# mkeeter/fidget

Measured on AMD Instinct MI355X. Metric: Mvoxel/s (interval+point eval) on prospero.vm 1024^3, higher is better.
Workload: dtype f32; 1 GPU; prospero.vm 3D heightmap+normals 1024^3, HipShape render hints (the library's tiles: 128/32/8, or 32/8 when the root level has few tiles), world_to_model=I

## Files before the change

fidget_amd/__init__.py:

```python
import ctypes as C
import math
import os
import re
import subprocess
import sys

import numpy as np

_HERE = os.path.dirname(os.path.abspath(__file__))
_CSRC = os.path.join(_HERE, "csrc")
LIB_PATH = os.environ.get("FHIP_LIB") or os.path.join(_CSRC, "libfidget_hip.so")
_SOURCES = ["capi.hip", "capi_core.hpp", "capi_context.hpp", "capi_tapes.hpp", "capi_eval.hpp", "capi_render.hpp", "frame_plan.hpp", "frame_schedule.hpp", "capi_effects.hpp", "capi_mesh.hpp", "capi_debug.hpp", "capi_solve.hpp", "solve.hip", "solve_lm.hpp", "kernels.hip", "prune2.hip", "effects.hip", "mesh.hip", "mesh_qef.hpp", "mesh_collapse.hpp", "mesh_edges.hpp", "mesh_walk.hpp", "mesh_split.hpp", "mesh_vox.hpp", "mesh_cc.hpp", "mesh_edt.hpp", "edt.hip", "capi_edt.hpp", "mesh_vmesh.hpp", "vmesh.hip", "capi_vmesh.hpp", "contour/contour.hpp", "host_mesh.hpp", "dev_ops.hpp", "host_graph.hpp", "host_regtape.hpp", "render_state.h", "tape_format.h",
            "gen_interp.py", "gen_tiles.py", "gen_tilesv.py", "gen_normals.py", "gen_prune.py", "gen_ubench.py", "gen_trans.py", "trans_funcs.hip", "trans_libm.hpp", "offsets.cpp", "../../include/fidget_hip.h",
            "../../include/fidget_hip_debug.h"]

UNARY = ["neg", "abs", "recip", "sqrt", "square", "floor", "ceil", "round", "sin", "cos", "tan",
         "asin", "acos", "atan", "exp", "ln", "not", "rand"]
BINARY = ["add", "sub", "mul", "div", "atan2", "min", "max", "compare", "mod", "and", "or", "mix"]

FH_OPS = (["Output", "Input", "CopyReg", "CopyImm"] + [u.capitalize() for u in UNARY]
          + [b.capitalize() + "RR" for b in ["add", "sub", "mul", "div", "atan2", "compare", "mix", "mod", "min", "max", "and", "or"]]
          + [b.capitalize() + "RI" for b in ["add", "sub", "mul", "div", "atan2", "compare", "mix", "mod", "min", "max", "and", "or"]]
          + [b.capitalize() + "IR" for b in ["sub", "div", "atan2", "compare", "mix", "mod"]])

STATUS = {1: "BadVarSlice", 2: "MismatchedSlices", 3: "BadChoiceSlice", 4: "MissingVar", 5: "BadTape",
          6: "Unsupported", 7: "HipError", 8: "Cancelled", 9: "ParseError", 10: "Overflow"}

VM_TILES_3D = [128, 64, 32, 16, 8]
VM_TILES_2D = [128, 32, 8]
GEOMETRY_PIXEL = np.dtype([("normal", np.float32, 3), ("depth", np.uint32)])
HIP_TILES_2D, HIP_TILES_3D = [128, 16], [128, 32, 8]
VM_TILES_2D, VM_TILES_3D = [128, 32, 8], [128, 64, 32, 16, 8]

EXPORTS = [
    "fhip_ctx_create", "fhip_ctx_destroy", "fhip_ctx_trim", "fhip_ctx_reserve_arena", "fhip_libm_probe", "fhip_last_error", "fhip_ctx_sync", "fhip_cancel", "fhip_cancel_reset", "fhip_cancel_watch", "fhip_ctx_set_option", "fhip_ctx_get_option",
    "fhip_tape_from_bytecode", "fhip_tape_free", "fhip_tape_len", "fhip_tape_reg_tape", "fhip_tape_choice_count", "fhip_tape_reg_count",
    "fhip_tape_var_count", "fhip_tape_output_count", "fhip_tape_ops", "fhip_simplify", "fhip_interval_eval",
    "fhip_point_eval", "fhip_float_eval", "fhip_grad_eval", "fhip_solve", "fhip_render2d", "fhip_render3d", "fhip_render3d_shard", "fhip_render3d_block", "fhip_merge_depth", "fhip_denoise_normals", "fhip_compute_ssao", "fhip_blur_ssao", "fhip_apply_shading", "fhip_to_rgba", "fhip_mesh_sample", "fhip_mesh_build", "fhip_mesh_vertices", "fhip_mesh_triangles", "fhip_mesh_vertices_ptr", "fhip_mesh_triangles_ptr", "fhip_mesh_free", "fhip_mesh_counts", "fhip_mesh_leaves", "fhip_mesh_sample_part", "fhip_mesh_part_bytes", "fhip_mesh_part_export", "fhip_mesh_merge", "fhip_mesh_vertices_dev", "fhip_mesh_triangles_dev", "fhip_mesh_stl_bytes", "fhip_mesh_stl", "fhip_mesh_vertex_grads", "fhip_shape_occupancy", "fhip_voxels_words", "fhip_shape_voxels", "fhip_voxels_slices", "fhip_voxels_layer_counts",
    "fhip_contour2d", "fhip_contours_counts", "fhip_contours_vertices", "fhip_contours_segments", "fhip_contours_next", "fhip_contours_vertices_dev", "fhip_contours_segments_dev", "fhip_contours_free", "fhip_contour_loops",
    "fhip_voxels_components", "fhip_components_counts", "fhip_components_table", "fhip_components_label_slices", "fhip_components_extract", "fhip_components_free",
    "fhip_voxels_distance", "fhip_distance_info", "fhip_distance_slices", "fhip_distance_dev", "fhip_distance_threshold", "fhip_distance_free",
    "fhip_voxels_surface", "fhip_voxels_mesh",
    "fhip_profile_enable", "fhip_profile_read", "fhip_profile_read_kernels", "fhip_render_counters", "fhip_graph_new", "fhip_graph_free",
    "fhip_graph_len", "fhip_graph_var", "fhip_graph_constant", "fhip_graph_unary", "fhip_graph_binary",
    "fhip_graph_from_text", "fhip_tape_from_graph", "fhip_tape_axis_slot", "fhip_tape_var_slot",
    "fhip_screen_to_world", "fhip_debug_groups", "fhip_debug_ubench", "fhip_debug_math_sweep", "fhip_debug_stats", "fhip_debug_leaf_stats", "fhip_debug_tape_links", "fhip_debug_tape_chain", "fhip_debug_bench", "fhip_debug_leaves", "fhip_debug_arena", "fhip_debug_probe", "fhip_debug_trans_probe", "fhip_debug_bound_tape", "fhip_debug_lane_frames", "fhip_debug_rare_frames", "fhip_debug_lane_tune", "fhip_debug_walk_dual", "fhip_debug_stl_pack", "fhip_tape_group_count", "fhip_tape_group_op",
    "fhip_tape_group", "fhip_tape_term_plan", "fhip_tape_term_group", "fhip_tape_term_tree", "fhip_tape_term_choice_src",
]


class FidgetHipError(RuntimeError):
    def __init__(self, status, msg=""):
        self.status = status
        super().__init__(f"{STATUS.get(status, status)}: {msg}")


def build(force=False, verbose=False):
    srcs = [os.path.join(_CSRC, s) for s in _SOURCES]
    if os.environ.get("FHIP_LIB"):
        return LIB_PATH
    if not force and os.path.exists(LIB_PATH) and all(os.path.getmtime(s) <= os.path.getmtime(LIB_PATH) for s in srcs):
        return LIB_PATH
    gen = os.path.join(_CSRC, "_gen")
    os.makedirs(gen, exist_ok=True)
    llvm = os.path.join(os.environ.get("ROCM_PATH", "/opt/rocm"), "lib", "llvm", "bin")
    co = os.path.join(gen, "interp_gfx950.co")

    def run(cmd, **kw):
        if verbose:
            print(" ".join(cmd))
        subprocess.check_call(cmd, **kw)

    run(["g++", "-std=c++17", "-I", _CSRC, os.path.join(_CSRC, "offsets.cpp"), "-o", os.path.join(gen, "offsets")])
    with open(os.path.join(gen, "offsets.json"), "w") as f:
        subprocess.check_call([os.path.join(gen, "offsets")], stdout=f)
    ll = os.path.join(gen, "trans_funcs.ll")
    run(["hipcc", "--offload-arch=gfx950", "-O3", "-std=c++17", "-ffp-contract=off", "-S", "-emit-llvm", "--cuda-device-only", "-I", _CSRC,
         "-o", ll, os.path.join(_CSRC, "trans_funcs.hip")])
    ir = open(ll).read()
    groups = set()
    for fn in ("fh_t_sin", "fh_t_atan2", "fh_t_mod", "fh_t_sin4", "fh_t_ln4"):
        m = re.search(rf"^define [^\n]*@{fn}\([^\n]*\) (#\d+)", ir, re.M)
        assert m, f"trans_funcs.ll: {fn} not found"
        groups.add(m.group(1))
    for g in groups:
        ir, n = re.subn(rf"^attributes {g} = {{ ", f'attributes {g} = {{ "amdgpu-num-sgpr"="18" ', ir, flags=re.M)
        assert n == 1
    with open(ll, "w") as f:
        f.write(ir)
    run([os.path.join(llvm, "llc"), "-mtriple=amdgcn-amd-amdhsa", "-mcpu=gfx950", "-O3", "-o", os.path.join(gen, "trans_funcs.s"), ll])
    run([sys.executable, os.path.join(_CSRC, "gen_interp.py"), os.path.join(gen, "offsets.json"),
         os.path.join(gen, "interp_gfx950.s"), os.path.join(gen, "trans_funcs.s")])
    run([os.path.join(llvm, "clang"), "-x", "assembler", "-target", "amdgcn-amd-amdhsa", "-mcpu=gfx950", "-c",
         os.path.join(gen, "interp_gfx950.s"), "-o", os.path.join(gen, "interp_gfx950.o")])
    run([os.path.join(llvm, "ld.lld"), "-shared", os.path.join(gen, "interp_gfx950.o"), "-o", co])
    run(["hipcc", "--offload-arch=gfx950", "-O3", "-std=c++17", "-ffp-contract=off", "-fPIC", "-shared",
         f'-DFH_INTERP_CO="{co}"', "-o", LIB_PATH, os.path.join(_CSRC, "capi.hip")])
    return LIB_PATH


class _Cfg2D(C.Structure):
    _fields_ = [("width", C.c_uint32), ("height", C.c_uint32), ("world_to_model", C.c_void_p), ("z", C.c_float),
                ("pixel_perfect", C.c_int), ("tile_sizes", C.c_void_p), ("n_tile_sizes", C.c_uint32),
                ("var_keys", C.c_void_p), ("var_values", C.c_void_p), ("n_vars", C.c_uint32),
                ("axis_slots", C.c_void_p)]


class _Cfg3D(C.Structure):
    _fields_ = [("width", C.c_uint32), ("height", C.c_uint32), ("depth", C.c_uint32), ("world_to_model", C.c_void_p),
                ("tile_sizes", C.c_void_p), ("n_tile_sizes", C.c_uint32), ("var_keys", C.c_void_p),
                ("var_values", C.c_void_p), ("n_vars", C.c_uint32), ("axis_slots", C.c_void_p)]


_lib = None


def lib():
    global _lib
    if _lib is None:
        if not os.path.exists(LIB_PATH):
            raise ImportError(f"{LIB_PATH} is missing: run `python -c 'import __graft_entry__ as g; g.build()'`")
        L = C.CDLL(LIB_PATH)
        vp, u32, i32, f32, u64 = C.c_void_p, C.c_uint32, C.c_int, C.c_float, C.c_uint64
        sig = {
            "fhip_ctx_create": (i32, [i32, vp, C.POINTER(vp)]), "fhip_ctx_destroy": (None, [vp]),
            "fhip_libm_probe": (i32, [C.c_char_p, C.c_size_t]), "fhip_ctx_trim": (i32, [vp]), "fhip_ctx_reserve_arena": (i32, [vp, C.c_size_t]),
            "fhip_last_error": (C.c_char_p, [vp]), "fhip_ctx_sync": (i32, [vp]),
            "fhip_cancel": (None, [vp]), "fhip_cancel_reset": (None, [vp]), "fhip_cancel_watch": (None, [vp, vp]),
            "fhip_ctx_set_option": (i32, [vp, C.c_char_p, i32]), "fhip_ctx_get_option": (i32, [vp, C.c_char_p, C.POINTER(i32)]),
            "fhip_tape_from_bytecode": (i32, [vp, vp, C.c_size_t, C.POINTER(vp)]), "fhip_tape_free": (None, [vp]),
            "fhip_tape_len": (u32, [vp]), "fhip_tape_reg_tape": (i32, [vp, u32, vp, u32, vp, u32, vp]), "fhip_tape_choice_count": (u32, [vp]), "fhip_tape_reg_count": (u32, [vp]),
            "fhip_tape_var_count": (u32, [vp]), "fhip_tape_output_count": (u32, [vp]),
            "fhip_tape_ops": (u32, [vp, vp, u32]),
            "fhip_simplify": (i32, [vp, vp, vp, u32, C.POINTER(vp)]),
            "fhip_interval_eval": (i32, [vp, vp, vp, u32, u32, vp, vp, vp]),
            "fhip_point_eval": (i32, [vp, vp, vp, u32, u32, vp, vp, vp]),
            "fhip_float_eval": (i32, [vp, vp, vp, vp, u32, vp]),
            "fhip_grad_eval": (i32, [vp, vp, vp, vp, u32, vp]),
            "fhip_solve": (i32, [vp, vp, u32, vp, vp, vp, u32, vp, u32, u32, vp, vp, vp, vp]),
            "fhip_render2d": (i32, [vp, vp, C.POINTER(_Cfg2D), vp, i32]),
            "fhip_render3d": (i32, [vp, vp, C.POINTER(_Cfg3D), vp, i32]),
            "fhip_render3d_shard": (i32, [vp, vp, C.POINTER(_Cfg3D), vp, i32, u32, u32]),
            "fhip_render3d_block": (i32, [vp, vp, C.POINTER(_Cfg3D), vp, i32, u32, vp]),
            "fhip_merge_depth": (i32, [vp, vp, vp, u64, u32]),
            "fhip_denoise_normals": (i32, [vp, vp, u32, u32, vp, i32]),
            "fhip_compute_ssao": (i32, [vp, vp, u32, u32, u32, vp, u32, vp, u32, vp, i32]),
            "fhip_blur_ssao": (i32, [vp, vp, u32, u32, vp, i32]),
            "fhip_apply_shading": (i32, [vp, vp, u32, u32, u32, vp, vp, i32]),
            "fhip_to_rgba": (i32, [vp, vp, u32, u32, i32, vp, i32]),
            "fhip_mesh_sample": (i32, [vp, vp, u32, vp, vp, vp, vp, u32, C.POINTER(vp)]), "fhip_mesh_free": (None, [vp]),
            "fhip_mesh_counts": (None, [vp, vp]), "fhip_mesh_leaves": (None, [vp, vp]),
            "fhip_mesh_build": (i32, [vp, vp, u32, vp, vp, vp, vp, u32, C.POINTER(vp)]),
            "fhip_mesh_vertices": (None, [vp, vp]), "fhip_mesh_triangles": (None, [vp, vp]),
            "fhip_mesh_vertices_ptr": (vp, [vp]), "fhip_mesh_triangles_ptr": (vp, [vp]),
            "fhip_mesh_sample_part": (i32, [vp, vp, u32, vp, vp, vp, vp, u32, u32, u32, C.POINTER(vp)]),
            "fhip_mesh_part_bytes": (C.c_uint64, [vp]), "fhip_mesh_part_export": (None, [vp, vp]),
            "fhip_mesh_merge": (i32, [vp, vp, vp, u32, vp, C.POINTER(vp)]),
            "fhip_mesh_vertices_dev": (vp, [vp]), "fhip_mesh_triangles_dev": (vp, [vp]),
            "fhip_mesh_stl_bytes": (u64, [vp]), "fhip_mesh_stl": (i32, [vp, vp, vp, i32]),
            "fhip_mesh_vertex_grads": (i32, [vp, vp, vp, vp, vp, vp, u32, vp, i32]),
            "fhip_shape_occupancy": (i32, [vp, vp, u32, vp, vp, vp, vp, u32, vp]),
            "fhip_voxels_words": (u64, [u32]), "fhip_shape_voxels": (i32, [vp, vp, u32, vp, vp, vp, vp, u32, vp, i32, vp]),
            "fhip_voxels_slices": (i32, [vp, vp, u32, u32, u32, vp, i32]), "fhip_voxels_layer_counts": (i32, [vp, vp, u32, vp, i32]),
            "fhip_contour2d": (i32, [vp, vp, vp, vp]), "fhip_contours_counts": (None, [vp, vp]), "fhip_contours_vertices": (i32, [vp, vp]),
            "fhip_contours_segments": (i32, [vp, vp]), "fhip_contours_next": (i32, [vp, vp]), "fhip_contours_vertices_dev": (vp, [vp]),
            "fhip_contours_segments_dev": (vp, [vp]), "fhip_contours_free": (None, [vp]), "fhip_contour_loops": (i32, [vp, u64, vp, vp, vp, vp]),
            "fhip_voxels_components": (i32, [vp, vp, u32, i32, u32, i32, vp]), "fhip_components_counts": (None, [vp, vp]),
            "fhip_components_table": (i32, [vp, vp, vp, vp, vp, vp]), "fhip_components_label_slices": (i32, [vp, vp, vp, i32, u32, u32, vp, i32]),
            "fhip_components_extract": (i32, [vp, vp, vp, i32, vp, u64, vp, i32]), "fhip_components_free": (None, [vp]),
            "fhip_voxels_distance": (i32, [vp, vp, u32, i32, i32, vp]), "fhip_distance_info": (None, [vp, vp]), "fhip_distance_slices": (i32, [vp, vp, u32, u32, vp, i32]),
            "fhip_distance_dev": (vp, [vp]), "fhip_distance_threshold": (i32, [vp, vp, u32, i32, vp, i32]), "fhip_distance_free": (None, [vp]),
            "fhip_voxels_surface": (i32, [vp, vp, u32, i32, vp]), "fhip_voxels_mesh": (i32, [vp, vp, u32, i32, vp]),
            "fhip_debug_stl_pack": (i32, [vp, vp, u64, vp, u64, vp]),
            "fhip_profile_enable": (None, [vp, i32]), "fhip_profile_read": (i32, [vp, vp, vp]), "fhip_profile_read_kernels": (i32, [vp, vp, vp]),
            "fhip_render_counters": (i32, [vp, vp]),
            "fhip_debug_stats": (i32, [vp, vp]), "fhip_debug_leaf_stats": (i32, [vp, vp]), "fhip_debug_tape_links": (u32, [vp, vp, u32]), "fhip_debug_tape_chain": (u32, [vp, vp, u32]),
            "fhip_tape_group_count": (u32, [vp]), "fhip_tape_group_op": (i32, [vp]),
            "fhip_tape_group": (i32, [vp, vp, u32, vp]), "fhip_tape_term_plan": (u32, [vp, vp]), "fhip_tape_term_group": (i32, [vp, vp, u32, vp]),
            "fhip_tape_term_tree": (u32, [vp, vp, u32]), "fhip_tape_term_choice_src": (u32, [vp, vp, u32]),
            "fhip_debug_leaves": (u32, [vp, vp, u32]), "fhip_debug_arena": (u32, [vp, u32, u32, vp]), "fhip_debug_probe": (i32, [vp, vp]),
            "fhip_debug_bench": (i32, [vp, vp, u32, u32, i32, vp]),
            "fhip_debug_walk_dual": (None, [vp, u64, vp, vp, u64, i32, vp, vp, vp]),
            "fhip_debug_groups": (u32, [vp, i32, u32, vp, u32, vp]),
            "fhip_debug_ubench": (i32, [vp, u32, u32, u32, vp]),
            "fhip_debug_math_sweep": (i32, [vp, i32, u32, u32, u64, vp, vp]),
            "fhip_debug_trans_probe": (i32, [vp, u32, u32, u32, u64, vp]),
            "fhip_debug_lane_frames": (u64, [vp]),
            "fhip_debug_rare_frames": (u64, [vp]),
            "fhip_debug_lane_tune": (i32, [vp, vp, vp]),
            "fhip_debug_bound_tape": (i32, [vp, vp, vp, vp, vp, u32, C.POINTER(vp)]),
            "fhip_graph_new": (vp, []), "fhip_graph_free": (None, [vp]), "fhip_graph_len": (u32, [vp]),
            "fhip_graph_var": (u32, [vp, i32, u64]), "fhip_graph_constant": (u32, [vp, f32]),
            "fhip_graph_unary": (u32, [vp, i32, u32]), "fhip_graph_binary": (u32, [vp, i32, u32, u32]),
            "fhip_graph_from_text": (u32, [vp, C.c_char_p]),
            "fhip_tape_from_graph": (i32, [vp, vp, vp, u32, C.POINTER(vp)]),
            "fhip_tape_axis_slot": (i32, [vp, i32]), "fhip_tape_var_slot": (i32, [vp, u64]),
            "fhip_screen_to_world": (None, [vp, i32, vp]),
        }
        for name, (res, args) in sig.items():
            fn = getattr(L, name)
            fn.restype = res
            fn.argtypes = args
        _lib = L
    return _lib


def _p(a):
    return a.ctypes.data_as(C.c_void_p) if a is not None else None


class HipContext:

    def __init__(self, device=0, stream=None):
        h = C.c_void_p()
        st = lib().fhip_ctx_create(device, C.c_void_p(stream or 0), C.byref(h))
        if st != 0:
            raise FidgetHipError(st, "no usable HIP device: fidget_amd has no CPU fallback")
        self._h = h

    def __del__(self):
        try:
            lib().fhip_ctx_destroy(self._h)
        except Exception:
            pass

    def check(self, st):
        if st != 0:
            raise FidgetHipError(st, (lib().fhip_last_error(self._h) or b"").decode())

    def sync(self):
        self.check(lib().fhip_ctx_sync(self._h))

    def trim(self):
        self.check(lib().fhip_ctx_trim(self._h))

    def reserve_arena(self, megabytes):
        self.check(lib().fhip_ctx_reserve_arena(self._h, int(megabytes)))

    def cancel(self):
        lib().fhip_cancel(self._h)

    def cancel_watch(self, flag):
        self._watched = flag
        lib().fhip_cancel_watch(self._h, None if flag is None else flag.ctypes.data_as(C.c_void_p))

    def cancel_reset(self):
        lib().fhip_cancel_reset(self._h)

    def lane_tune(self):
        ms, ln = (C.c_float * 3)(), C.c_int(0)
        ph = lib().fhip_debug_lane_tune(self._h, ms, C.byref(ln))
        return {"phase": int(ph), "stage_pipeline_ms": [float(ms[0]), float(ms[2])], "frame_lanes_ms": float(ms[1]), "kept": "frame lanes" if ln.value else "stage pipeline"}

    def lane_frames(self):
        return int(lib().fhip_debug_lane_frames(self._h))

    def rare_frames(self):
        return int(lib().fhip_debug_rare_frames(self._h))

    def set_option(self, name, value=1):
        self.check(lib().fhip_ctx_set_option(self._h, name.encode(), int(value)))

    def option(self, name):
        v = C.c_int(0)
        self.check(lib().fhip_ctx_get_option(self._h, name.encode(), C.byref(v)))
        return v.value

    def options(self, **kw):
        import contextlib

        @contextlib.contextmanager
        def scope():
            old = {k: self.option(k) for k in kw}
            try:
                for k, v in kw.items():
                    self.set_option(k, v)
                yield self
            finally:
                for k, v in old.items():
                    self.set_option(k, v)
        return scope()

    def profile(self, on):
        lib().fhip_profile_enable(self._h, int(on))

    def profile_read(self):
        ms = np.zeros(4, np.float64)
        n = np.zeros(4, np.uint32)
        self.check(lib().fhip_profile_read(self._h, _p(ms), _p(n)))
        names = ["tiles", "points", "normals", "other"]
        return {k: (float(ms[i]), int(n[i])) for i, k in enumerate(names)}

    def profile_read_kernels(self):
        ms = np.zeros(8, np.float64)
        n = np.zeros(8, np.uint32)
        self.check(lib().fhip_profile_read_kernels(self._h, _p(ms), _p(n)))
        names = ["fh_columns", "fh_float_eval_16x4", "fh_float_eval_32x2", "fh_tiles", "fh_prune1", "fh_tiles_v32", "fh_tiles_v64", "unused"]
        return {k: (float(ms[i]), int(n[i])) for i, k in enumerate(names)}

    def counters(self):
        c = np.zeros(8, np.uint64)
        self.check(lib().fhip_render_counters(self._h, _p(c)))
        return {"arena_ops": int(c[0]), "arena_overflow": int(c[1]), "leaves_last_slab": int(c[2]),
                "queue_overflow": int(c[3]), "groups_last_slab": [int(v) for v in c[4:6]], "hip_tile_stage_frames": int(c[6]), "substituted_tile_lists": int(c[7])}

    def last_leaves(self, cap=1 << 20):
        dt = np.dtype([("off", np.uint32), ("len", np.uint32), ("regs", np.uint16), ("choices", np.uint16),
                       ("x", np.uint32), ("y", np.uint32), ("z", np.uint32)])
        buf = np.zeros(cap, dt)
        n = lib().fhip_debug_leaves(self._h, _p(buf), cap)
        return buf[:n]

    def groups(self, kind, index, cap=1 << 20):
        dt = np.dtype([("off", np.uint32), ("len", np.uint32), ("regs", np.uint16), ("choices", np.uint16),
                       ("x", np.uint32), ("y", np.uint32), ("z", np.uint32), ("first", np.uint32), ("n", np.uint32), ("stride", np.uint32)])
        assert dt.itemsize == 36
        buf = np.zeros(cap, dt)
        cnt = np.zeros(2, np.uint32)
        n = lib().fhip_debug_groups(self._h, kind, index, _p(buf), cap, _p(cnt))
        return buf[:n], (int(cnt[0]), int(cnt[1]))

    def arena_ops(self, off, n):
        buf = np.zeros(n, np.uint64)
        got = lib().fhip_debug_arena(self._h, int(off), int(n), _p(buf))
        return buf[:got]

    def leaf_stats(self):
        c = np.zeros(8, np.uint64)
        self.check(lib().fhip_debug_leaf_stats(self._h, _p(c)))
        return {"leaves": int(c[0]), "tape_ops": int(c[1]), "tape_words_read": int(c[2]), "lane_ops": int(c[3]),
                "prune2_phase_clocks_max": [int(v) for v in c[4:8]]}

    def wave_stats(self):
        c = np.zeros(64, np.uint64)
        self.check(lib().fhip_debug_stats(self._h, _p(c)))
        names = ["tiles_l0", "tiles_l1", "tiles_l2", "tiles_l3", "tiles_l4", "columns_c0", "columns_c12", "tiles_2d"]
        self.tile_v = {f"l{l}": {"slots": int(c[8 + l]), "fwd_clocks": int(c[16 + l]), "prune_clocks": int(c[24 + l]), "max_slot_clocks": int(c[l])}
                       for l in range(8) if c[8 + l]}
        self.tile_phases = {f"l{l}": {"fwd_us": int(c[32 + l]) / 100.0, "prune_us": int(c[40 + l]) / 100.0,
                                      "ops": int(c[48 + l]), "ops_written": int(c[56 + l]), "fwd_shader_clocks": int(c[16 + l])} for l in range(8) if c[48 + l]}
        return {k: {"busy_us_sum": int(c[4 * i]) / 100.0, "busy_us_max": int(c[4 * i + 1]) / 100.0,
                    "waves": int(c[4 * i + 2]), "units": int(c[4 * i + 3])} for i, k in enumerate(names) if c[4 * i + 2]}


_default_ctx = None


def default_context():
    global _default_ctx
    if _default_ctx is None:
        _default_ctx = HipContext(int(os.environ.get("LOCAL_RANK", "0")) if os.environ.get("FHIP_USE_LOCAL_RANK") else 0)
    return _default_ctx


BAD_NODE = 0xFFFFFFFF


class BadNode(Exception):
    pass


class Node(int):
    pass


class Context:

    def __init__(self):
        self._h = C.c_void_p(lib().fhip_graph_new())

    def __del__(self):
        try:
            lib().fhip_graph_free(self._h)
        except Exception:
            pass

    def __len__(self):
        return lib().fhip_graph_len(self._h)

    def _node(self, v):
        if isinstance(v, (float, int)) and not isinstance(v, Node):
            return self.constant(float(v))
        return v

    def x(self): return Node(lib().fhip_graph_var(self._h, 0, 0))
    def y(self): return Node(lib().fhip_graph_var(self._h, 1, 0))
    def z(self): return Node(lib().fhip_graph_var(self._h, 2, 0))
    def var(self, index): return Node(lib().fhip_graph_var(self._h, 3, int(index)))
    def constant(self, f): return Node(lib().fhip_graph_constant(self._h, float(f)))

    def _un(self, name, a):
        r = lib().fhip_graph_unary(self._h, UNARY.index(name), int(self._node(a)))
        if r == BAD_NODE:
            raise BadNode()
        return Node(r)

    def _bin(self, name, a, b):
        r = lib().fhip_graph_binary(self._h, BINARY.index(name), int(self._node(a)), int(self._node(b)))
        if r == BAD_NODE:
            raise BadNode()
        return Node(r)

    def less_than(self, lhs, rhs):
        return self.max(self._bin("compare", rhs, lhs), 0.0)

    def less_than_or_equal(self, lhs, rhs):
        return self.min(self.add(self._bin("compare", rhs, lhs), 1.0), 1.0)

    def if_nonzero_else(self, cond, a, b):
        cond, a, b = self._node(cond), self._node(a), self._node(b)
        lhs = self.and_(cond, a)
        rhs = self.and_(self.not_(cond), b)
        return self.or_(lhs, rhs)

    @staticmethod
    def from_text(text):
        ctx = Context()
        if isinstance(text, str):
            text = text.encode()
        r = lib().fhip_graph_from_text(ctx._h, text)
        if r == BAD_NODE:
            raise ValueError("parse error")
        return ctx, Node(r)


def _mk_un(name):
    def f(self, a):
        return self._un(name, a)
    return f


def _mk_bin(name):
    def f(self, a, b):
        return self._bin(name, a, b)
    return f


for _n in UNARY:
    setattr(Context, {"not": "not_"}.get(_n, _n), _mk_un(_n))
for _n in BINARY:
    setattr(Context, {"and": "and_", "or": "or_", "mod": "modulo"}.get(_n, _n), _mk_bin(_n))


class Shape:

    def __init__(self, ctx=None, node=None, n_regs=255, _h=None, roots=None, hip=None, _vars=None):
        self._hip = hip
        self.n_regs = n_regs
        if _h is not None:
            self._h = _h
            self._vars = _vars
            return
        if roots is None:
            roots = [node]
        r = np.array([int(n) for n in roots], dtype=np.uint32)
        h = C.c_void_p()
        st = lib().fhip_tape_from_graph(None, ctx._h, _p(r), len(r), C.byref(h))
        if st != 0:
            raise FidgetHipError(st, "tape construction failed")
        self._h = h
        self._vars = None

    @property
    def hip(self):
        if self._hip is None:
            self._hip = default_context()
        return self._hip

    def __del__(self):
        try:
            lib().fhip_tape_free(self._h)
        except Exception:
            pass

    def groups(self):
        n = lib().fhip_tape_group_count(self._h)
        out = []
        for g in range(n):
            h = C.c_void_p()
            st = lib().fhip_tape_group(None, self._h, g, C.byref(h))
            if st != 0:
                raise FidgetHipError(st, "tape group")
            out.append(Shape(_h=h, hip=self._hip, _vars=self._vars))
        op = lib().fhip_tape_group_op(self._h)
        return ({30: "min", 31: "max"}.get(op, ""), out)

    def term_parts(self):
        n = self.term_plan()
        gs = []
        for g in range(n["groups"]):
            h = C.c_void_p()
            st = lib().fhip_tape_term_group(None, self._h, g, C.byref(h))
            if st != 0:
                raise FidgetHipError(st, "term group")
            gs.append(Shape(_h=h, hip=self._hip, _vars=self._vars))
        tree = np.zeros((max(n["tree_ops"], 1), 3), np.uint32)
        lib().fhip_tape_term_tree(self._h, _p(tree), n["tree_ops"])
        src = np.zeros(max(n["choices"], 1), np.uint32)
        lib().fhip_tape_term_choice_src(self._h, _p(src), n["choices"])
        return gs, tree[:n["tree_ops"]], src[:n["choices"]]

    def term_plan(self):
        info = (C.c_uint32 * 4)()
        n = lib().fhip_tape_term_plan(self._h, info)
        return dict(groups=n, terms=info[0], tree_ops=info[1], tree_regs=info[2], choices=info[3])

    @staticmethod
    def from_vm(path_or_text, n_regs=255, hip=None):
        text = open(path_or_text).read() if os.path.exists(path_or_text) else path_or_text
        ctx, root = Context.from_text(text)
        return Shape(ctx, root, n_regs, hip=hip)

    @staticmethod
    def from_bytecode(words, axis_slots=(0, 1, 2), hip=None):
        w = np.ascontiguousarray(words, dtype=np.uint32)
        h = C.c_void_p()
        st = lib().fhip_tape_from_bytecode(None, _p(w), len(w), C.byref(h))
        if st != 0:
            raise FidgetHipError(st, "bad bytecode")
        return Shape(_h=h, hip=hip, _vars=tuple(axis_slots))

    def device_len(self): return lib().fhip_tape_len(self._h)

    def size(self):
        if self.n_regs == 255 and lib().fhip_tape_reg_count(self._h) <= 255:
            return self.device_len()
        return int(self.reg_tape()[1][0])
    __len__ = size
    def ssa_len(self): return self.device_len()

    def reg_tape(self, n_regs=None, want_words=False):
        n_regs = self.n_regs if n_regs is None else n_regs
        info = np.zeros(4, np.uint32)
        st = lib().fhip_tape_reg_tape(self._h, n_regs, None, 0, None, 0, _p(info))
        if st not in (0, 6):
            raise FidgetHipError(st, "register allocation")
        n = int(info[0])
        rec = np.zeros((n, 4), np.uint32)
        words = np.zeros(2 * n + 4, np.uint32)
        st = lib().fhip_tape_reg_tape(self._h, n_regs, _p(rec), n, _p(words), len(words), _p(info))
        if want_words and st == 6:
            raise ValueError("ReservedRegister")
        NAMES = ["Output", "Input", "CopyReg", "CopyImm", "Neg", "Abs", "Recip", "Sqrt", "Square", "Floor", "Ceil", "Round", "Sin", "Cos", "Tan",
                 "Asin", "Acos", "Atan", "Exp", "Ln", "Not", "Rand"]
        BIN = ["Add", "Sub", "Mul", "Div", "Atan2", "Compare", "Mix", "Mod", "Min", "Max", "And", "Or"]
        ops = []
        for op, o, a, w in rec.tolist():
            if op == 52: ops.append(("Load", "", o, 0, 0, w, 0))
            elif op == 53: ops.append(("Store", "", 0, a, 0, w, 0))
            elif op == 0: ops.append(("Output", "", 0, a, 0, w, 0))
            elif op == 1: ops.append(("Input", "", o, 0, 0, w, 0))
            elif op == 3: ops.append(("CopyImm", "", o, 0, 0, 0, w))
            elif op < 22: ops.append((NAMES[op], "Reg", o, a, 0, 0, 0))
            elif op < 34: ops.append((BIN[op - 22], "RegReg", o, a, w, 0, 0))
            elif op < 46: ops.append((BIN[op - 34], "RegImm", o, a, 0, 0, w))
            else: ops.append((["Sub", "Div", "Atan2", "Compare", "Mix", "Mod"][op - 46], "ImmReg", o, a, 0, 0, w))
        out = (ops, tuple(int(v) for v in info))
        return out + (words,) if want_words else out
# ... 1114 lines not shown
```

fidget_amd/csrc/capi.hip:

```cpp
#include <hip/hip_runtime.h>
#include <ctype.h>
#include <stdio.h>
#include <stdlib.h>
#include <string.h>

#include <algorithm>
#include <atomic>
#include <chrono>
#include <mutex>
#include <string>
#include <functional>
#include <memory>
#include <vector>

#include "../../include/fidget_hip.h"
#include "../../include/fidget_hip_debug.h"
#include "host_graph.hpp"
#include "host_regtape.hpp"
#include "kernels.hip"
#include "effects.hip"
#include "mesh.hip"
#include "prune2.hip"
#include "solve.hip"
#include "host_mesh.hpp"
#include "frame_schedule.hpp"

#include "capi_core.hpp"

extern "C" {

#include "capi_context.hpp"
#include "capi_tapes.hpp"
#include "capi_eval.hpp"
#include "capi_bound.hpp"
#include "capi_render.hpp"
#include "capi_effects.hpp"
#include "capi_mesh.hpp"
#include "capi_solve.hpp"
#include "capi_debug.hpp"

}
```

fidget_amd/csrc/capi_core.hpp:

```cpp
struct DevBuf {
    void* p = nullptr;
    size_t cap = 0;
    hipError_t ensure(size_t bytes) {
        if (bytes <= cap) return hipSuccess;
        if (p) (void)hipFree(p);
        p = nullptr; cap = 0;
        hipError_t e = hipMalloc(&p, bytes);
        if (e == hipSuccess) cap = bytes;
        return e;
    }
    void release() { if (p) (void)hipFree(p); p = nullptr; cap = 0; }
};

static std::atomic<uint64_t> g_tape_serial{1};
struct BoundCache {
    struct Entry {
        uint64_t hash = 0, used = 0;
        std::vector<uint64_t> key;
        std::shared_ptr<const fhip_tape> tape;
    };
    std::mutex lock;
    std::vector<Entry> entries;
    uint64_t clock = 0;
};
struct fhip_tape {
    const uint64_t serial = g_tape_serial.fetch_add(1);
    fh::HostTape t;
    mutable uint64_t* d_ops = nullptr;
    std::vector<fh::HostTape> groups;
    int group_op = -1;
    fh::TermPlan plan;
    std::vector<fh::HostTape> tgroups;
    mutable FhTopOp* d_top = nullptr;
    mutable uint32_t* d_chsrc = nullptr;
    mutable uint64_t* d_links = nullptr;
    mutable uint64_t* d_ctab = nullptr;
    mutable std::atomic<uint32_t> input_slots{0x80000000u};
    mutable uint32_t n_chain = 0;
    mutable bool links_tried = false;
    mutable std::mutex upload_lock;
    mutable int device = -1;
    uint64_t parent_serial = 0;
    std::weak_ptr<const fhip_tape> self;
    mutable BoundCache bound;
};
struct fhip_graph {
    fh::Graph g;
};

#ifndef __HIP_DEVICE_COMPILE__
__asm__(".section .rodata\n.global fh_interp_co\n.p2align 6\nfh_interp_co:\n.incbin \"" FH_INTERP_CO "\"\n.previous\n");
#endif
extern "C" const char fh_interp_co[];
enum { FH_ASM_COLUMNS = 0, FH_ASM_FLOAT_16x4, FH_ASM_FLOAT_32x2, FH_ASM_TILES, FH_ASM_PRUNE1, FH_ASM_TILES_V32, FH_ASM_TILES_V64, FH_ASM_PROBE, FH_ASM_UBENCH, FH_ASM_COLUMNS_T, FH_ASM_NORMALS, FH_ASM_NORMALS_T, FH_ASM_TILES_T, FH_ASM_TILES_V32_T, FH_ASM_TILES_V64_T, FH_ASM_FLOAT_16x4_T, FH_ASM_FLOAT_32x2_T, FH_ASM_TRANS_PROBE, FH_ASM_COUNT };
static const char* const FH_ASM_NAMES[FH_ASM_COUNT] = {"fh_columns", "fh_float_eval_16x4", "fh_float_eval_32x2", "fh_tiles", "fh_prune1",
                                                       "fh_tiles_v32", "fh_tiles_v64", "fh_probe", "fh_ubench", "fh_columns_t", "fh_normals", "fh_normals_t", "fh_tiles_t", "fh_tiles_v32_t", "fh_tiles_v64_t", "fh_float_eval_16x4_t", "fh_float_eval_32x2_t", "fh_trans_probe"};

#define FH_OPTION_LIST(X)                                                                                                       \
     \
    X(no_asm, 0) X(no_split, 0) X(no_asm_tiles, 0) X(no_tiles_v, 0) X(no_asm_tiles_t, 0) X(no_columns_t, 0) X(no_asm_normals, 0)   \
    X(no_tape_groups, 0) X(prune2, 1)                                                                                           \
                      \
    X(no_column_inv, 0) X(no_zrep, 0) X(root32_max, 4096) X(column_walk, 1) X(column_group, 2)                                                    \
                                                                                                 \
    X(no_pipeline, 0) X(frame_lanes, 4) X(lanes_fail, 0) X(slab_layers, 4) X(arena_mb, 4096)  \
          \
    X(mesh_device_assembly, 1) X(mesh_device_walk, 1) X(mesh_simplify_min_ops, 256) X(mesh_keep_device, 0)                      \
                                                                                                              \
    X(probe, 0) X(stats, 0)
struct FhOptions {
#define X(name, dflt) int name = dflt;
    FH_OPTION_LIST(X)
#undef X
};
struct FhOptionEntry { const char* name; int FhOptions::*field; };
static const FhOptionEntry FH_OPTION_TABLE[] = {
#define X(name, dflt) {#name, &FhOptions::name},
    FH_OPTION_LIST(X)
#undef X
};
static void options_from_env(FhOptions& o) {
    for (const FhOptionEntry& e : FH_OPTION_TABLE) {
        std::string var = "FHIP_";
        for (const char* c = e.name; *c; c++) var += (char)toupper((unsigned char)*c);
        if (const char* v = getenv(var.c_str())) o.*(e.field) = *v ? atoi(v) : 1;
    }
}

struct FrameBufs {
    DevBuf state, arena, leaves, leaf_table, zbuf, normals, fp_lists, mind, squeue, slots[2], leaves_b, leaf_table_b, fp_lists_b, chw[2], tvals, topch, chwr, gscratch, rare_scratch;
    DevBuf queue[FH_MAX_LEVELS];
    uint32_t frame_stamp = 0;
    uint64_t resident_serial = 0;
    uint32_t resident_groups = 0;
    uint32_t forked = 0;
    bool async_pending = false;
    hipEvent_t ev_done = nullptr;
    bool ev_done_valid = false;
    std::shared_ptr<const fhip_tape> bound_hold;
    void release_all() {
        DevBuf* bufs[] = {&state, &arena, &leaves, &leaf_table, &zbuf, &normals, &fp_lists, &mind, &squeue, &slots[0], &slots[1],
                          &leaves_b, &leaf_table_b, &fp_lists_b, &chw[0], &chw[1], &tvals, &topch, &chwr, &gscratch, &rare_scratch};
        for (DevBuf* b : bufs) b->release();
        for (auto& q : queue) q.release();
        if (ev_done) (void)hipEventDestroy(ev_done);
        ev_done = nullptr;
        bound_hold.reset();
    }
};
struct fhip_ctx : FrameBufs {
    FhOptions opt;
#define FH_EXTRA_SETS 4
    FrameBufs others[FH_EXTRA_SETS];
    uint32_t extra_sets = 3;
    bool frame_pipeline = true;
    hipStream_t stream_pre = nullptr;
    uint32_t pre_turn = 0;
    hipEvent_t ev_rest_fork = nullptr, ev_rest_join = nullptr;
    hipEvent_t ev_pre = nullptr, ev_l0 = nullptr, ev_l1 = nullptr;
    hipModule_t asm_mod = nullptr;
    hipFunction_t asm_fn[FH_ASM_COUNT] = {};
    bool use_asm = true;
    bool probe = false;
    bool use_split = true;
    bool use_pipeline = true;
    hipStream_t stream2 = nullptr, stream3 = nullptr;
    std::vector<hipEvent_t> ev_tiles, ev_leaves, ev_aux;
    hipEvent_t ev_fork = nullptr;
    FhRenderState last_state_b;
    uint32_t slab_contexts = 4;
    int device = 0;
    hipStream_t stream = nullptr;
    int n_cu = 256;
    std::string err;
    bool launch_failed = false;
    std::atomic<int> cancelled{0};
    const std::atomic<int>* cancel_src = nullptr;
    std::atomic<const volatile unsigned char*> watch{nullptr};
    bool is_cancelled() const {
        if ((cancel_src ? cancel_src : &cancelled)->load() != 0) return true;
        const volatile unsigned char* w = watch.load(std::memory_order_relaxed);
        return w && *w != 0;
    }
    DevBuf tmp_out, io_a, io_b, io_c, io_d, io_e;
    DevBuf sticky;
    struct Staging { void* p = nullptr; size_t cap = 0; hipEvent_t ev = nullptr; bool used = false; } staging[8];
    DevBuf mesh_leaves;
    void* mesh_pinned = nullptr;
    size_t mesh_pinned_cap = 0;
    void* mesh_octree_cache = nullptr;
    uint32_t* mesh_first = nullptr;
    size_t mesh_first_cap = 0;
    uint32_t staging_next = 0;
    size_t arena_bytes = (size_t)256 << 20, arena_cap_bytes = (size_t)4 << 30;
    uint64_t hip_tile_frames = 0;
    uint64_t substituted_tiles = 0;
    int last_hip_error = 0;
    volatile uint32_t* host_flags = nullptr;
    bool profiling = false;
    std::vector<std::pair<int, std::pair<hipEvent_t, hipEvent_t>>> prof_events;
    std::vector<std::pair<int, std::pair<hipEvent_t, hipEvent_t>>> asm_events;
    FhRenderState last_state;
    bool have_last_state = false;
    std::vector<fhip_ctx*> lanes;
    uint32_t lane_next = 0;
    uint64_t rare_frames = 0;
    uint64_t lane_frames = 0;
    uint64_t lane_frames_wanted = 0;
    hipEvent_t ev_last = nullptr;
    bool ev_last_valid = false;
    struct LaneTune {
        uint64_t key = 0, used = 0;
        int phase = 0;
        uint32_t n = 0;
        bool lanes = false;
        float ms[3] = {0.0f, 0.0f, 0.0f};
        hipEvent_t ev[6] = {nullptr, nullptr, nullptr, nullptr, nullptr, nullptr};
    };
    std::vector<LaneTune> lane_tune;
    uint64_t tune_last_key = 0, tune_clock = 0;
    int tune_cur = -1;
    bool is_lane = false, lane_stream_owned = false;
    DevBuf lane_img;
    hipEvent_t lane_done = nullptr, lane_copied = nullptr;
    bool lane_copied_valid = false;
};

#define FH_ARENA_START_MB 128
static void apply_options(fhip_ctx* c) {
    c->use_asm = c->opt.no_asm == 0;
    c->use_split = c->opt.no_split == 0;
    c->probe = c->opt.probe != 0;
    c->use_pipeline = c->opt.no_pipeline == 0;
    c->frame_pipeline = true;
    c->slab_contexts = 4;
    c->arena_cap_bytes = (size_t)std::max(1, c->opt.arena_mb) << 20;
    c->arena_bytes = std::min(c->arena_cap_bytes, std::max(c->arena_bytes, (size_t)FH_ARENA_START_MB << 20));
    c->extra_sets = 3;
}

static fhip_status finish_render(fhip_ctx* ctx);
static void mesh_cache_release(void* octree);
static fhip_status fail(fhip_ctx* ctx, fhip_status s, const std::string& msg) {
    if (ctx) ctx->err = msg;
    return s;
}
#define HIP_TRY(ctx, call)                                                                                       \
    do {                                                                                                         \
        hipError_t e_ = (call);                                                                                  \
        if (e_ != hipSuccess) {                                                                                  \
            if (ctx) (ctx)->last_hip_error = (int)e_;                                                            \
            return fail(ctx, FHIP_ERR_HIP, std::string(#call) + ": " + hipGetErrorString(e_));                   \
        }                                                                                                        \
    } while (0)

template <class F>
static void launch(fhip_ctx* ctx, hipStream_t st, int klass, F&& f) {
    if (ctx->profiling) {
        hipEvent_t a, b;
        (void)hipEventCreate(&a);
        (void)hipEventCreate(&b);
        (void)hipEventRecord(a, st);
        f();
        (void)hipEventRecord(b, st);
        ctx->prof_events.push_back({klass, {a, b}});
    } else {
        f();
    }
}

static bool simplify_host(const fh::HostTape& p, const uint8_t* choices, fh::HostTape& out) {
    std::vector<int> map(FH_MAX_REGS, -1);
    fh::RegPool pool;
    std::vector<uint64_t> rev;
    uint32_t ci = p.n_choices, kept = 0;
    auto use = [&](uint32_t r) { if (map[r] < 0) map[r] = pool.take(); return (uint32_t)map[r]; };
    for (size_t k = p.ops.size(); k-- > 0;) {
        const uint64_t w = p.ops[k];
        const uint32_t w0 = (uint32_t)w, w1 = (uint32_t)(w >> 32);
        const uint32_t op = FH_W_OP(w0), ro = FH_W_OUT(w0), ra = FH_W_A(w0), rb = w1;
        const bool is_choice = fh_is_choice(op);
        uint32_t c = FH_CHOICE_BOTH;
        if (is_choice) {
            c = choices[--ci];
            if (c == FH_CHOICE_UNKNOWN) return false;
        }
        if (op == FH_OUTPUT) { rev.push_back(fh_pack(op, 0, use(ra), 0, w1)); continue; }
        const int no = map[ro];
        if (no < 0) continue;
        map[ro] = -1;
        int alias = -1;
        bool copy_imm = false;
        if (op == FH_COPY_REG) alias = (int)ra;
        else if (is_choice && c == FH_CHOICE_LEFT) alias = (int)ra;
        else if (is_choice && c == FH_CHOICE_RIGHT) { if (fh_is_rr(op)) alias = (int)rb; else copy_imm = true; }
        if (alias >= 0) {
            if (map[alias] < 0) { map[alias] = no; continue; }
            pool.give(no);
            rev.push_back(fh_pack(FH_COPY_REG, no, map[alias], 0, 0));
            continue;
        }
        pool.give(no);
        if (copy_imm) { rev.push_back(fh_pack(FH_COPY_IMM, no, 0, 0, w1)); continue; }
        uint32_t na = 0, nb = 0;
        if (op != FH_INPUT && op != FH_COPY_IMM) na = use(ra);
        if (fh_is_rr(op)) nb = use(rb);
        if (is_choice) kept++;
        rev.push_back(fh_pack(op, no, na, nb, w1));
    }
    out.ops.assign(rev.rbegin(), rev.rend());
    out.n_regs = pool.high;
    out.n_choices = kept;
    out.n_outputs = p.n_outputs;
    out.n_vars = p.n_vars;
    out.vars = p.vars;
    return true;
}

template <class T> struct FhKArgs;
template <class... K> struct FhKArgs<void (*)(K...)> {
    template <class... A> static size_t pack(char* buf, A&&... a) {
        size_t off = 0;
        auto put = [&](auto v) {
            constexpr size_t al = alignof(decltype(v));
            off = (off + al - 1) & ~(al - 1);
            memcpy(buf + off, &v, sizeof(v));
            off += sizeof(v);
        };
        (put(static_cast<K>(std::forward<A>(a))), ...);
        return off;
    }
    static constexpr size_t bytes = (sizeof(K) + ... + 0) + 16 * sizeof...(K);
};
template <auto Kernel, class... A>
static inline void fh_launch(fhip_ctx* ctx, dim3 g, dim3 b, size_t lds, hipStream_t st, A&&... a) {
    constexpr int MAXDEV = 64;
    static std::atomic<hipFunction_t> fns[MAXDEV];
    static std::atomic<bool> no_handle[MAXDEV];
    const int device = ctx->device;
    hipFunction_t fn = nullptr;
    if (device >= 0 && device < MAXDEV) {
        fn = fns[device].load(std::memory_order_acquire);
        if (!fn && !no_handle[device].load(std::memory_order_relaxed)) {
            if (hipGetFuncBySymbol(&fn, (const void*)Kernel) != hipSuccess || !fn) { fn = nullptr; no_handle[device].store(true, std::memory_order_relaxed); (void)hipGetLastError(); }
            else fns[device].store(fn, std::memory_order_release);
        }
    }
    hipError_t e;
    if (!fn) {
        hipLaunchKernelGGL(Kernel, g, b, lds, st, std::forward<A>(a)...);
        e = hipGetLastError();
    } else {
        alignas(16) char buf[FhKArgs<decltype(Kernel)>::bytes];
        size_t bytes = FhKArgs<decltype(Kernel)>::pack(buf, std::forward<A>(a)...);
        void* extra[] = {HIP_LAUNCH_PARAM_BUFFER_POINTER, buf, HIP_LAUNCH_PARAM_BUFFER_SIZE, &bytes, HIP_LAUNCH_PARAM_END};
        e = hipModuleLaunchKernel(fn, g.x, g.y, g.z, b.x, b.y, b.z, (unsigned)lds, st, nullptr, extra);
    }
    if (e != hipSuccess) {
        ctx->launch_failed = true;
        ctx->last_hip_error = (int)e;
        if (ctx->err.empty()) ctx->err = std::string("kernel launch: ") + hipGetErrorString(e);
        (void)hipGetLastError();
    }
}
#define FH_KLAUNCH(kernel, grid, block, lds, stream, ...) fh_launch<kernel>(ctx, grid, block, lds, stream, ##__VA_ARGS__)
```

fidget_amd/csrc/capi_debug.hpp:

```cpp
void fhip_profile_enable(fhip_ctx* ctx, int on) { ctx->profiling = on != 0; }
fhip_status fhip_profile_read(fhip_ctx* ctx, double ms[4], uint32_t launches[4]) {
    HIP_TRY(ctx, hipStreamSynchronize(ctx->stream));
    for (int i = 0; i < 4; i++) { ms[i] = 0; launches[i] = 0; }
    for (auto& e : ctx->prof_events) {
        float t = 0;
        if (hipEventElapsedTime(&t, e.second.first, e.second.second) == hipSuccess) { ms[e.first] += t; launches[e.first]++; }
    }
    return FHIP_OK;
}
fhip_status fhip_profile_read_kernels(fhip_ctx* ctx, double ms[8], uint32_t launches[8]) {
    HIP_TRY(ctx, hipStreamSynchronize(ctx->stream));
    for (int i = 0; i < 8; i++) { ms[i] = 0; launches[i] = 0; }
    for (auto& e : ctx->asm_events) {
        float t = 0;
        if (e.first < 8 && hipEventElapsedTime(&t, e.second.first, e.second.second) == hipSuccess) { ms[e.first] += t; launches[e.first]++; }
    }
    return FHIP_OK;
}
fhip_status fhip_render_counters(fhip_ctx* ctx, uint64_t out[8]) {
    fhip_status st = finish_render(ctx);
    if (st != FHIP_OK && st != FHIP_ERR_OVERFLOW) return st;
    const FhRenderState& S = ctx->last_state;
    out[0] = S.arena_head; out[1] = S.arena_overflow; out[2] = S.n_leaves; out[3] = S.queue_overflow;
    for (int i = 0; i < 2; i++) out[4 + i] = S.count[i + 1];
    out[6] = ctx->hip_tile_frames;
    out[7] = ctx->substituted_tiles;
    return FHIP_OK;
}

fhip_status fhip_debug_stats(fhip_ctx* ctx, uint64_t out[64]) {
    fhip_status st = finish_render(ctx);
    if (st != FHIP_OK && st != FHIP_ERR_OVERFLOW) return st;
    for (int i = 0; i < 64; i++) out[i] = ctx->last_state.stat[i];
    return FHIP_OK;
}
uint32_t fhip_debug_tape_links(const fhip_tape* tape, uint64_t* out, uint32_t cap) {
    std::vector<uint64_t> lk;
    std::vector<uint64_t> cops;
    if (!fh::compute_links(tape->t, lk, cops)) return 0;
    for (size_t i = 0; i < lk.size() && i < cap; i++) out[i] = lk[i];
    return (uint32_t)lk.size();
}
uint32_t fhip_debug_tape_chain(const fhip_tape* tape, uint32_t* out, uint32_t cap) {
    std::vector<uint64_t> lk;
    std::vector<uint64_t> cops;
    if (!fh::compute_links(tape->t, lk, cops)) return 0;
    const std::vector<uint32_t> chain = chain_table(tape, cops);
    for (size_t i = 0; i < chain.size() && i < cap; i++) out[i] = chain[i];
    return (uint32_t)chain.size();
}
fhip_status fhip_debug_leaf_stats(fhip_ctx* ctx, uint64_t out[8]) {
    fhip_status st = finish_render(ctx);
    if (st != FHIP_OK && st != FHIP_ERR_OVERFLOW) return st;
    for (int i = 0; i < 8; i++) out[i] = ctx->last_state.leaf_stat[i];
    return FHIP_OK;
}

uint32_t fhip_debug_leaves(fhip_ctx* ctx, void* out, uint32_t cap) {
    if (finish_render(ctx) != FHIP_OK) return 0;
    const uint32_t n = std::min(std::min(ctx->last_state.n_leaves, ctx->last_state.leaf_cap), cap);
    if (hipMemcpy(out, ctx->last_state.leaves, (size_t)n * sizeof(FhLeaf), hipMemcpyDeviceToHost) != hipSuccess) return 0;
    return n;
}

uint32_t fhip_debug_groups(fhip_ctx* ctx, int kind, uint32_t index, void* out, uint32_t cap, uint32_t counts[2]) {
    counts[0] = counts[1] = 0;
    if (finish_render(ctx) != FHIP_OK) return 0;
    const FhRenderState& S = ctx->last_state;
    const FhGroup* base; uint32_t ns, nb, qcap;
    if (kind == 0) {
        if (index >= FH_MAX_LEVELS || !S.queue[index]) return 0;
        base = S.queue[index]; ns = S.count[index]; nb = S.count_big[index]; qcap = S.qcap[index];
    } else {
        if (index >= FH_MAX_SLABS || !S.squeue) return 0;
        base = S.squeue + (size_t)index * S.squeue_cap; ns = S.scount[index]; nb = S.scount_big[index]; qcap = S.squeue_cap;
    }
    ns = std::min(ns, qcap); nb = std::min(nb, qcap - ns);
    const uint32_t n0 = std::min(ns, cap), n1 = std::min(nb, cap - n0);
    if (n0 && hipMemcpy(out, base, (size_t)n0 * sizeof(FhGroup), hipMemcpyDeviceToHost) != hipSuccess) return 0;
    if (n1 && hipMemcpy((FhGroup*)out + n0, base + (qcap - nb), (size_t)n1 * sizeof(FhGroup), hipMemcpyDeviceToHost) != hipSuccess) return 0;
    counts[0] = n0; counts[1] = n1;
    return n0 + n1;
}

fhip_status fhip_debug_probe(fhip_ctx* ctx, float* out) {
    HIP_TRY(ctx, ctx->io_a.ensure(16 * 256));
    struct { void* p; } ka = {ctx->io_a.p};
    if (launch_asm(ctx, ctx->stream, FH_ASM_PROBE, 1, &ka, sizeof(ka)) != hipSuccess) return FHIP_ERR_HIP;
    HIP_TRY(ctx, hipStreamSynchronize(ctx->stream));
    HIP_TRY(ctx, hipMemcpy(out, ctx->io_a.p, 16 * 256, hipMemcpyDeviceToHost));
    return FHIP_OK;
}

fhip_status fhip_debug_ubench(fhip_ctx* ctx, uint32_t test, uint32_t iters, uint32_t n_waves, float* out) {
    HIP_TRY(ctx, ctx->io_a.ensure((size_t)n_waves * 4));
    HIP_TRY(ctx, hipMemsetAsync(ctx->io_a.p, 0, (size_t)n_waves * 4, ctx->stream));
    struct { void* p; uint32_t test, iters; } ka = {ctx->io_a.p, test, iters};
    if (launch_asm(ctx, ctx->stream, FH_ASM_UBENCH, n_waves, &ka, sizeof(ka), 64) != hipSuccess) return FHIP_ERR_HIP;
    HIP_TRY(ctx, hipStreamSynchronize(ctx->stream));
    HIP_TRY(ctx, hipMemcpy(out, ctx->io_a.p, (size_t)n_waves * 4, hipMemcpyDeviceToHost));
    return FHIP_OK;
}

fhip_status fhip_debug_math_sweep(fhip_ctx* ctx, int op, uint32_t first, uint32_t stride, uint64_t n, const float* ref, uint64_t out[4]) {
    (void)hipSetDevice(ctx->device);
    HIP_TRY(ctx, ctx->io_a.ensure(n * 4));
    HIP_TRY(ctx, ctx->io_b.ensure(64));
    HIP_TRY(ctx, hipMemcpyAsync(ctx->io_a.p, ref, n * 4, hipMemcpyHostToDevice, ctx->stream));
    HIP_TRY(ctx, hipMemsetAsync(ctx->io_b.p, 0, 64, ctx->stream));
    hipLaunchKernelGGL(k_math_sweep, dim3(ctx->n_cu * 16), dim3(256), 0, ctx->stream, op, first, stride, (size_t)n, (const float*)ctx->io_a.p,
                       (unsigned long long*)ctx->io_b.p);
    HIP_TRY(ctx, hipGetLastError());
    unsigned long long r[4];
    HIP_TRY(ctx, hipMemcpyAsync(r, ctx->io_b.p, 32, hipMemcpyDeviceToHost, ctx->stream));
    HIP_TRY(ctx, hipStreamSynchronize(ctx->stream));
    out[0] = r[0] >> 32; out[1] = r[1]; out[2] = r[2]; out[3] = r[0] & 0xFFFFFFFFull;
    return FHIP_OK;
}

fhip_status fhip_debug_trans_probe(fhip_ctx* ctx, uint32_t copy, uint32_t fn, uint32_t first, uint64_t n, uint64_t out[2]) {
    (void)hipSetDevice(ctx->device);
    if (!n || n % 256 || n > (1ull << 28)) return fail(ctx, FHIP_ERR_UNSUPPORTED, "trans probe: n must be a multiple of 256, at most 2^28");
    if (!ctx->asm_fn[FH_ASM_TRANS_PROBE]) return fail(ctx, FHIP_ERR_UNSUPPORTED, "trans probe: the assembly kernels are not loaded");
    HIP_TRY(ctx, ctx->io_a.ensure(n * 4));
    HIP_TRY(ctx, ctx->io_b.ensure(64));
    HIP_TRY(ctx, hipMemsetAsync(ctx->io_a.p, 0x5A, n * 4, ctx->stream));
    HIP_TRY(ctx, hipMemsetAsync(ctx->io_b.p, 0, 64, ctx->stream));
    struct { void* out; uint32_t first, copy, fn, pad; } ka = {ctx->io_a.p, first, copy, fn, 0};
    if (launch_asm(ctx, ctx->stream, FH_ASM_TRANS_PROBE, (uint32_t)(n / 256), &ka, sizeof(ka)) != hipSuccess) return FHIP_ERR_HIP;
    hipLaunchKernelGGL(k_trans_compare, dim3(ctx->n_cu * 16), dim3(256), 0, ctx->stream, (int)fn, first, (size_t)n, (const uint32_t*)ctx->io_a.p,
                       (unsigned long long*)ctx->io_b.p);
    HIP_TRY(ctx, hipGetLastError());
    unsigned long long r[2];
    HIP_TRY(ctx, hipMemcpyAsync(r, ctx->io_b.p, 16, hipMemcpyDeviceToHost, ctx->stream));
    HIP_TRY(ctx, hipStreamSynchronize(ctx->stream));
    out[0] = r[1]; out[1] = r[0] & 0xFFFFFFFFull;
    return FHIP_OK;
}

uint64_t fhip_debug_rare_frames(const fhip_ctx* ctx) {
    if (!ctx) return 0;
    uint64_t n = ctx->rare_frames;
    for (const fhip_ctx* l : ctx->lanes) n += l ? l->rare_frames : 0;
    return n;
}
uint64_t fhip_debug_lane_frames(const fhip_ctx* ctx) { return ctx ? ctx->lane_frames : 0; }
int fhip_debug_lane_tune(const fhip_ctx* ctx, float ms[3], int* lanes) {
    if (!ctx) return -1;
    for (const auto& t : ctx->lane_tune)
        if (t.key == ctx->tune_last_key) {
            if (ms) { ms[0] = t.ms[0]; ms[1] = t.ms[1]; ms[2] = t.ms[2]; }
            if (lanes) *lanes = t.lanes ? 1 : 0;
            return t.phase;
        }
    return -1;
}

uint32_t fhip_debug_arena(fhip_ctx* ctx, uint32_t off, uint32_t n, uint64_t* out) {
    if ((size_t)(off + (size_t)n) * 8 > ctx->arena_bytes) return 0;
    if (hipMemcpy(out, (const uint64_t*)ctx->arena.p + off, (size_t)n * 8, hipMemcpyDeviceToHost) != hipSuccess) return 0;
    return n;
}

fhip_status fhip_debug_bench(fhip_ctx* ctx, const fhip_tape* tape, uint32_t n_waves, uint32_t reps, int variant, double* ms) {
    fhip_status st = tape_to_device(ctx, tape);
    if (st) return st;
    HIP_TRY(ctx, ctx->state.ensure(2 * sizeof(FhRenderState)));
    FhRenderState S;
    memset(&S, 0, sizeof(S));
    for (int i = 0; i < FH_MAX_INPUTS; i++) S.P.in_kind[i] = i % 3;
    HIP_TRY(ctx, hipMemcpy(ctx->state.p, &S, sizeof(S), hipMemcpyHostToDevice));
    HIP_TRY(ctx, ctx->io_a.ensure((size_t)n_waves * WAVE * 4));
    hipEvent_t a, b;
    HIP_TRY(ctx, hipEventCreate(&a));
    HIP_TRY(ctx, hipEventCreate(&b));
    const uint32_t len = (uint32_t)tape->t.ops.size();
    FhRenderState* dS = (FhRenderState*)ctx->state.p;
    for (int it = 0; it < 2; it++) {
        HIP_TRY(ctx, hipEventRecord(a, ctx->stream));
        if (variant == 0) hipLaunchKernelGGL((k_bench_points<16, 4>), dim3(n_waves), dim3(WAVE), 0, ctx->stream, dS, tape->d_ops, len, reps, (float*)ctx->io_a.p);
        else if (variant == 1) hipLaunchKernelGGL((k_bench_points<32, 2>), dim3(n_waves), dim3(WAVE), 0, ctx->stream, dS, tape->d_ops, len, reps, (float*)ctx->io_a.p);
        else if (variant == 3) hipLaunchKernelGGL((k_bench_points<32, 1>), dim3(n_waves), dim3(WAVE), 0, ctx->stream, dS, tape->d_ops, len, reps, (float*)ctx->io_a.p);
        else hipLaunchKernelGGL((k_bench_points<0, 1>), dim3(n_waves), dim3(WAVE), (size_t)std::max<uint32_t>(tape->t.n_regs, 1) * WAVE * 4, ctx->stream, dS, tape->d_ops, len, reps, (float*)ctx->io_a.p);
        HIP_TRY(ctx, hipEventRecord(b, ctx->stream));
        HIP_TRY(ctx, hipEventSynchronize(b));
    }
    float t = 0;
    HIP_TRY(ctx, hipEventElapsedTime(&t, a, b));
    *ms = t;
    (void)hipEventDestroy(a); (void)hipEventDestroy(b);
    return FHIP_OK;
}

static const int UNARY_MAP[] = {FH_NEG, FH_ABS, FH_RECIP, FH_SQRT, FH_SQUARE, FH_FLOOR, FH_CEIL, FH_ROUND, FH_SIN,
                                FH_COS, FH_TAN, FH_ASIN, FH_ACOS, FH_ATAN, FH_EXP, FH_LN, FH_NOT, FH_RAND};
static const int BINARY_MAP[] = {FH_ADD_RR, FH_SUB_RR, FH_MUL_RR, FH_DIV_RR, FH_ATAN2_RR, FH_MIN_RR, FH_MAX_RR,
                                 FH_COMPARE_RR, FH_MOD_RR, FH_AND_RR, FH_OR_RR, FH_MIX_RR};
fhip_graph* fhip_graph_new(void) { return new fhip_graph(); }
void fhip_graph_free(fhip_graph* g) { delete g; }
uint32_t fhip_graph_len(const fhip_graph* g) { return (uint32_t)g->g.nodes.size(); }
uint32_t fhip_graph_var(fhip_graph* g, int kind, uint64_t index) { return g->g.var((uint8_t)kind, kind < 3 ? 0 : index); }
uint32_t fhip_graph_constant(fhip_graph* g, float v) { return g->g.constant(v); }
uint32_t fhip_graph_unary(fhip_graph* g, int opcode, uint32_t a) {
    if (opcode < 0 || opcode >= 18) return fh::NO_NODE;
    return g->g.unary(UNARY_MAP[opcode], a);
}
uint32_t fhip_graph_binary(fhip_graph* g, int opcode, uint32_t a, uint32_t b) {
    if (opcode < 0 || opcode >= 12) return fh::NO_NODE;
    return g->g.binary(BINARY_MAP[opcode], a, b);
}
uint32_t fhip_graph_from_text(fhip_graph* g, const char* text) {
    std::string err;
    return g->g.parse(text, err);
}
```

fidget_amd/csrc/capi_render.hpp:

```cpp
static fhip_status bind_inputs(fhip_ctx* ctx, const fhip_tape* tape, const int32_t* axis_slots, const uint64_t* keys,
                               const float* vals, uint32_t n, FhRender& P) {
    const fh::HostTape& t = tape->t;
    std::vector<char> bound(FH_MAX_INPUTS, 0);
    for (uint32_t s = 0; s < FH_MAX_INPUTS; s++) { P.in_kind[s] = 3; P.in_value[s] = 0.0f; }
    for (int a = 0; a < 3; a++) {
        const int s = axis_slots ? axis_slots[a] : t.vars.axis[a];
        if (s >= 0 && s < FH_MAX_INPUTS) { P.in_kind[s] = (uint32_t)a; bound[s] = 1; }
    }
    for (uint32_t i = 0; i < n; i++) {
        const int s = axis_slots ? (int)keys[i] : t.vars.slot_of(3, keys[i]);
        if (s >= 0 && s < FH_MAX_INPUTS) { P.in_value[s] = vals[i]; bound[s] = 1; }
    }
    for (uint32_t s = 0; s < t.n_vars; s++)
        if (!bound[s]) return fail(ctx, FHIP_ERR_MISSING_VAR, "a variable of the shape has no value");
    return FHIP_OK;
}

struct HostSpans {
    double t[8] = {0, 0, 0, 0, 0, 0, 0, 0};
    uint64_t n = 0;
    std::chrono::steady_clock::time_point last;
    void start() { last = std::chrono::steady_clock::now(); }
    void mark(int k) { const auto now = std::chrono::steady_clock::now(); t[k] += std::chrono::duration<double, std::micro>(now - last).count(); last = now; }
    void frame() {
        if (++n % 200 == 0) {
            fprintf(stderr, "fidget-hip host us per frame: set-up %.1f prepare %.1f upload %.1f coarse %.1f slabs %.1f finish %.1f\n", t[0] / 200, t[1] / 200, t[2] / 200, t[3] / 200, t[4] / 200, t[5] / 200);
            for (double& x : t) x = 0;
        }
    }
};
static thread_local HostSpans g_spans;
#define FH_SPAN(k) do { if (ctx->opt.stats & 2) g_spans.mark(k); } while (0)

static PlanInputs plan_inputs(const fhip_ctx* ctx) {
    PlanInputs in;
    in.slab_layers = ctx->opt.slab_layers; in.no_zrep = ctx->opt.no_zrep; in.no_column_inv = ctx->opt.no_column_inv; in.no_columns_t = ctx->opt.no_columns_t;
    in.no_asm_normals = ctx->opt.no_asm_normals; in.no_asm_tiles = ctx->opt.no_asm_tiles; in.no_asm_tiles_t = ctx->opt.no_asm_tiles_t;
    in.no_tape_groups = ctx->opt.no_tape_groups; in.prune2 = ctx->opt.prune2; in.root32_max = ctx->opt.root32_max;
    in.use_asm = ctx->use_asm; in.use_split = ctx->use_split; in.n_cu = (uint32_t)ctx->n_cu; in.slab_contexts = ctx->slab_contexts; in.arena_bytes = ctx->arena_bytes;
    return in;
}

static hipError_t sync_own_streams(fhip_ctx* ctx) {
    hipError_t e = hipSuccess;
    for (hipStream_t s : {ctx->stream, ctx->stream2, ctx->stream3, ctx->stream_pre}) {
        const hipError_t r = hipStreamSynchronize(s);
        if (r != hipSuccess && e == hipSuccess) e = r;
    }
    for (fhip_ctx* L : ctx->lanes)
        if (L) { const hipError_t r = sync_own_streams(L); if (r != hipSuccess && e == hipSuccess) e = r; }
    return e;
}
static fhip_status grow_arena_if_asked(fhip_ctx* ctx, size_t want) {
    if (want == ctx->arena_bytes) return FHIP_OK;
    HIP_TRY(ctx, sync_own_streams(ctx));
    if (ctx->host_flags) ctx->host_flags[0] = 0;
    ctx->arena_bytes = want;
    return FHIP_OK;
}

static fhip_status ensure_root_tables(fhip_ctx* ctx, const fhip_tape* tape) {
    const fh::HostTape& t = tape->t;
    std::lock_guard<std::mutex> guard(tape->upload_lock);
    if (tape->device >= 0 && tape->device != ctx->device) return fail(ctx, FHIP_ERR_UNSUPPORTED, "this tape's device copies belong to another device: build the tape per device");
    tape->device = ctx->device;
    if (!tape->d_top) {
        static_assert(sizeof(FhTopOp) == sizeof(fh::TopOp), "top op layout");
        HIP_TRY(ctx, hipMalloc((void**)&tape->d_top, tape->plan.top.size() * sizeof(FhTopOp)));
        HIP_TRY(ctx, hipMemcpy(tape->d_top, tape->plan.top.data(), tape->plan.top.size() * sizeof(FhTopOp), hipMemcpyHostToDevice));
        HIP_TRY(ctx, hipMalloc((void**)&tape->d_chsrc, std::max<size_t>(tape->plan.choice_src.size(), 1) * 4));
        HIP_TRY(ctx, hipMemcpy(tape->d_chsrc, tape->plan.choice_src.data(), tape->plan.choice_src.size() * 4, hipMemcpyHostToDevice));
    }
    if (ctx->opt.prune2 && !tape->links_tried) {
        tape->links_tried = true;
        std::vector<uint64_t> lk;
        std::vector<uint64_t> cops;
        if (fh::compute_links(t, lk, cops)) {
            uint64_t *dl = nullptr, *dc = nullptr;
            std::vector<uint32_t> chain = chain_table(tape, cops);
            const size_t n_cops = std::max<size_t>(cops.size(), 1);
            cops.resize(n_cops + (chain.size() + 1) / 2, 0);
            if (!chain.empty()) memcpy(cops.data() + n_cops, chain.data(), chain.size() * 4);
            hipError_t e = hipMalloc((void**)&dl, lk.size() * 8);
            if (e == hipSuccess) e = hipMemcpy(dl, lk.data(), lk.size() * 8, hipMemcpyHostToDevice);
            if (e == hipSuccess) e = hipMalloc((void**)&dc, std::max<size_t>(cops.size(), 1) * 8);
            if (e == hipSuccess) e = hipMemcpy(dc, cops.data(), cops.size() * 8, hipMemcpyHostToDevice);
            if (e != hipSuccess) {
                if (dl) (void)hipFree(dl);
                if (dc) (void)hipFree(dc);
                HIP_TRY(ctx, e);
            }
            tape->d_links = dl; tape->d_ctab = dc; tape->n_chain = (uint32_t)chain.size();
        }
    }
    return FHIP_OK;
}

static void bind_state(fhip_ctx* ctx, const fhip_tape* tape, bool is3d, RenderSetup& R) {
    FhRenderState& S = R.S;
    const FhRender& P = S.P;
    S.frame_stamp = ++ctx->frame_stamp;
    if (R.hip_tiles_unasked) ctx->hip_tile_frames++;
    S.gscratch = R.big_hbm ? (char*)ctx->gscratch.p : nullptr;
    if (is3d) {
        uint32_t* mp = (uint32_t*)ctx->mind.p;
        for (uint32_t l = 0; l < P.n_levels; l++) {
            S.mind[l] = mp;
            mp += (size_t)((P.width + P.tiles[l] - 1) / P.tiles[l]) * ((P.height + P.tiles[l] - 1) / P.tiles[l]);
        }
        for (int c = 0; c < 3; c++) S.fp_list[c] = (uint32_t*)ctx->fp_lists.p + (size_t)c * R.n_footprints;
        S.hit_list = (uint32_t*)ctx->fp_lists.p + (size_t)3 * R.n_footprints;
    }
    S.arena = (uint64_t*)ctx->arena.p;
    S.arena_overflow = 0;
    for (int l = 0; l < FH_MAX_LEVELS; l++) {
        S.queue[l] = (FhGroup*)ctx->queue[l].p;
        S.count[l] = S.cursor[l] = S.count_big[l] = S.cursor_big[l] = 0;
    }
    S.count_big[0] = (uint32_t)R.roots.size();
    if (R.groups) {
        S.ttop = tape->d_top; S.chsrc = tape->d_chsrc;
        R.d_ctab = tape->d_ctab; R.d_links = tape->d_links;
        S.tvals = (float*)ctx->tvals.p; S.topch = (uint8_t*)ctx->topch.p; S.chwr = (uint32_t*)ctx->chwr.p;
    }
    if (R.prune1) for (int k = 0; k < 2; k++) S.chw[k] = (uint32_t*)ctx->chw[k].p;
    if (R.split) for (int k = 0; k < 2; k++) S.slots[k] = (FhSlot*)ctx->slots[k].p;
    S.squeue = (FhGroup*)ctx->squeue.p;
    for (int k = 0; k < FH_MAX_SLABS; k++) S.scount[k] = S.scount_big[k] = 0;
    S.queue_overflow = 0;
    S.leaves = (FhLeaf*)ctx->leaves.p;
    S.n_leaves = S.leaf_cursor = S.leaf_cursor_big = S.normal_cursor = S.normal_cursor_big = 0;
    S.leaf_table = (FhLeafRef*)ctx->leaf_table.p;
    for (int c = 0; c < 3; c++) S.fp_count[c] = S.fp_cursor[c] = 0;
    S.zbuf = (uint64_t*)ctx->zbuf.p;
    S.normals = (float*)ctx->normals.p;
    S.image2d = nullptr;
    memset(S.stat, 0, sizeof(S.stat));
    memset(S.leaf_stat, 0, sizeof(S.leaf_stat));
    S.want_stats = (ctx->profiling || ctx->probe || (ctx->opt.stats & 1)) ? 1 : 0;
}

static fhip_status prepare(fhip_ctx* ctx, const fhip_tape* tape, const TapeFacts& facts, bool is3d, const std::vector<uint32_t>& ts,
                           const PartSpec& part, RenderSetup& R) {
    static_assert(PLAN_BAD_TAPE == FHIP_ERR_BAD_TAPE && PLAN_UNSUPPORTED == FHIP_ERR_UNSUPPORTED, "the plan's refusals are fhip_status values");
    const FhRender& P = R.S.P;
    PlanInputs in = plan_inputs(ctx);
    in.arena_bytes = arena_bytes_for(ctx->arena_bytes, ctx->arena_cap_bytes, (size_t)FH_ARENA_START_MB << 20, ctx->host_flags && ctx->host_flags[0] != 0, facts.n_ops,
                                     is3d && !R.root_invariant ? (uint64_t)P.width * P.height * P.depth : 0);
    const PlanStatus ps = plan_frame(facts, in, is3d, ts, part, R);
    if (ps.status) return fail(ctx, (fhip_status)ps.status, ps.msg);
    { const fhip_status gs = grow_arena_if_asked(ctx, in.arena_bytes); if (gs) return gs; }
    const FrameBytes& B = R.bytes;
    HIP_TRY(ctx, ctx->gscratch.ensure(B.gscratch));
    HIP_TRY(ctx, ctx->state.ensure(4 * sizeof(FhRenderState)));
    { void* const before = ctx->arena.p; HIP_TRY(ctx, ctx->arena.ensure(ctx->arena_bytes)); if (ctx->arena.p != before) ctx->resident_serial = 0; }
    for (size_t l = 0; l < ts.size(); l++) HIP_TRY(ctx, ctx->queue[l].ensure(B.queue[l]));
    const std::pair<DevBuf*, size_t> list[] = {{&ctx->squeue, B.squeue}, {&ctx->leaves, B.leaves}, {&ctx->leaves_b, B.leaves_b}, {&ctx->leaf_table, B.leaf_table},
                                               {&ctx->leaf_table_b, B.leaf_table_b}, {&ctx->zbuf, B.zbuf}, {&ctx->normals, B.normals}, {&ctx->fp_lists, B.fp_lists},
                                               {&ctx->fp_lists_b, B.fp_lists_b}, {&ctx->mind, B.mind}, {&ctx->tvals, B.tvals}, {&ctx->topch, B.topch}, {&ctx->chwr, B.chwr},
                                               {&ctx->chw[0], B.chw[0]}, {&ctx->chw[1], B.chw[1]}, {&ctx->slots[0], B.slots}, {&ctx->slots[1], B.slots}};
    for (const auto& b : list) HIP_TRY(ctx, b.first->ensure(b.second));
    if (R.groups) {
        const fhip_status us = ensure_root_tables(ctx, tape);
        if (us) return us;
        plan_linked_prune(facts, in, tape->d_links && tape->d_ctab, tape->n_chain, R);
    }
    bind_state(ctx, tape, is3d, R);
    return FHIP_OK;
}

static int blocks_for(const fhip_ctx* ctx, size_t lds, int max_per_cu);
static int blocks_big(const fhip_ctx* ctx, const RenderSetup& R, size_t lds, int max_per_cu) {
    return R.big_hbm ? (int)R.hbm_waves : blocks_for(ctx, lds, max_per_cu);
}
static int blocks_for(const fhip_ctx* ctx, size_t lds, int max_per_cu) {
    int per_cu = lds ? (int)std::min<size_t>((size_t)max_per_cu, FH_LDS_MAX / std::max<size_t>(lds, 1)) : max_per_cu;
    per_cu = std::max(per_cu, 1);
    return ctx->n_cu * per_cu;
}

static fhip_status finish_render(fhip_ctx* ctx) {
    HIP_TRY(ctx, hipMemcpyAsync(&ctx->last_state, ctx->state.p, sizeof(FhRenderState), hipMemcpyDeviceToHost, ctx->stream));
    HIP_TRY(ctx, hipStreamSynchronize(ctx->stream));
    for (uint32_t k = 1; k < ctx->forked; k++) {
        HIP_TRY(ctx, hipMemcpy(&ctx->last_state_b, (char*)ctx->state.p + k * sizeof(FhRenderState), sizeof(FhRenderState), hipMemcpyDeviceToHost));
        ctx->last_state.queue_overflow += ctx->last_state_b.queue_overflow;
        ctx->last_state.arena_overflow += ctx->last_state_b.arena_overflow;
        for (int i = 0; i < 64; i++) ctx->last_state.stat[i] += ctx->last_state_b.stat[i];
        for (int i = 0; i < 8; i++) ctx->last_state.leaf_stat[i] += ctx->last_state_b.leaf_stat[i];
    }
    ctx->have_last_state = true;
    if (ctx->last_state.queue_overflow) return fail(ctx, FHIP_ERR_OVERFLOW, "device work queue overflow");
    return FHIP_OK;
}

struct FrameClear { void* p = nullptr; size_t bytes = 0; uint32_t fill = 0; };
static fhip_status upload_frame(fhip_ctx* ctx, hipStream_t st, const fhip_tape* tape, RenderSetup& R, const FrameClear (&clear)[3]) {
    const size_t roots_bytes = R.roots.size() * sizeof(FhGroup);
    fhip_ctx::Staging& sg = ctx->staging[ctx->staging_next++ % 8];
    if (sg.ev && sg.used) HIP_TRY(ctx, hipEventSynchronize(sg.ev));
    if (!sg.ev) HIP_TRY(ctx, hipEventCreateWithFlags(&sg.ev, hipEventDisableTiming));
    if (sg.cap < sizeof(FhRenderState) + roots_bytes) {
        if (sg.p) (void)hipHostFree(sg.p);
        sg.p = nullptr; sg.cap = 0;
        HIP_TRY(ctx, hipHostMalloc(&sg.p, sizeof(FhRenderState) + roots_bytes + 4096, hipHostMallocDefault));
        sg.cap = sizeof(FhRenderState) + roots_bytes + 4096;
    }
    memcpy(sg.p, &R.S, sizeof(FhRenderState));
    if (roots_bytes) memcpy((char*)sg.p + sizeof(FhRenderState), R.roots.data(), roots_bytes);
    { const fhip_status hs = hold_bound(ctx, tape); if (hs) return hs; }
    if (ctx->resident_serial != tape->serial || ctx->resident_groups != R.S.n_tgroups) {
        ctx->resident_serial = 0;
        HIP_TRY(ctx, hipMemcpyAsync(ctx->arena.p, tape->t.ops.data(), tape->t.ops.size() * 8, hipMemcpyHostToDevice, st));
        for (uint32_t g = 0; g < R.S.n_tgroups; g++)
            HIP_TRY(ctx, hipMemcpyAsync((uint64_t*)ctx->arena.p + R.S.tgroup[g].off, tape->tgroups[g].ops.data(),
                                        tape->tgroups[g].ops.size() * 8, hipMemcpyHostToDevice, st));
        ctx->resident_serial = tape->serial;
        ctx->resident_groups = R.S.n_tgroups;
    }
    static_assert(sizeof(FhRenderState) % 4 == 0 && sizeof(FhGroup) % 4 == 0, "copied as 32-bit words");
    FhFrameBegin fb;
    memset(&fb, 0, sizeof(fb));
    fb.state_dst = (uint32_t*)ctx->state.p; fb.state_src = (const uint32_t*)sg.p; fb.state_words = (uint32_t)(sizeof(FhRenderState) / 4);
    if (!R.roots.empty()) {
        fb.roots_dst = (uint32_t*)((FhGroup*)ctx->queue[0].p + (R.S.qcap[0] - R.roots.size()));
        fb.roots_src = (const uint32_t*)((const char*)sg.p + sizeof(FhRenderState));
        fb.roots_words = (uint32_t)(roots_bytes / 4);
    }
    size_t most = 0;
    for (int k = 0; k < 3; k++) {
        fb.clear[k] = (uint32_t*)clear[k].p; fb.clear_words[k] = clear[k].bytes / 4; fb.fill[k] = clear[k].fill;
        if (clear[k].p) most = std::max(most, clear[k].bytes);
    }
    const unsigned blocks = (unsigned)std::max<size_t>(8, std::min<size_t>((size_t)ctx->n_cu * 32, (most + 64 * 64 - 1) / (64 * 64)));
    FH_KLAUNCH(k_frame_begin, dim3(blocks), dim3(WAVE), 0, st, fb);
    HIP_TRY(ctx, hipGetLastError());
    HIP_TRY(ctx, hipEventRecord(sg.ev, st));
    sg.used = true;
    for (auto& e : ctx->prof_events) { (void)hipEventDestroy(e.second.first); (void)hipEventDestroy(e.second.second); }
    ctx->prof_events.clear();
    for (auto& e : ctx->asm_events) { (void)hipEventDestroy(e.second.first); (void)hipEventDestroy(e.second.second); }
    ctx->asm_events.clear();
    return FHIP_OK;
}

#define FH_LAUNCH_TILES(IS3D, FULL, BIG, grid, lds)                                                                  \
    do {                                                                                                            \
        if (R.tl == 64) FH_KLAUNCH((k_tiles<IS3D, FULL, BIG, 64>), dim3(grid), dim3(WAVE), lds, st, dS, level); \
        else FH_KLAUNCH((k_tiles<IS3D, FULL, BIG, 16>), dim3(grid), dim3(WAVE), lds, st, dS, level);            \
    } while (0)
struct KaTiles { FhRenderState* S; uint32_t level, big, max_regs, max_choices, n_waves, flags, skip_regs, skip_choices; };
struct KaPrune1 { FhRenderState* S; uint32_t level, big, max_choices, mode; };
struct KaColumns { FhRenderState* S; uint32_t n_waves, slots, depmask, flags, pad[2]; const void* table; uint32_t nfpl, layers; };
struct KaNormals { FhRenderState* S; uint32_t n_waves, slots, z_lo, z_hi, bucket_cap, mode; };

struct FrameStreams { hipStream_t s[N_ROLES]; Role cur; hipStream_t on() const { return s[cur]; } };
static FrameStreams frame_streams(const fhip_ctx* ctx, Role at = CALLER) { return FrameStreams{{ctx->stream, ctx->stream_pre, ctx->stream2, ctx->stream3}, at}; }
static hipError_t hop(FrameStreams& fs, Role to, hipEvent_t ev) {
    if (to == fs.cur) return hipSuccess;
    const hipError_t e = hipEventRecord(ev, fs.on());
    fs.cur = to;
    return e != hipSuccess ? e : hipStreamWaitEvent(fs.on(), ev, 0);
}
static ScheduleInputs schedule_inputs(const fhip_ctx* ctx, int out_is_device) {
    ScheduleInputs in;
    in.no_tiles_v = ctx->opt.no_tiles_v; in.no_zrep = ctx->opt.no_zrep; in.column_walk = ctx->opt.column_walk; in.column_group = ctx->opt.column_group;
    in.frame_pipeline = ctx->frame_pipeline; in.use_pipeline = ctx->use_pipeline; in.profiling = ctx->profiling; in.slab_contexts = ctx->slab_contexts;
    in.has_side = ctx->stream2 != nullptr; in.has_tail = ctx->stream3 != nullptr; in.has_flags = ctx->host_flags != nullptr; in.out_is_device = out_is_device != 0;
    return in;
}
static char* rare_file(const fhip_ctx* ctx, const FhRenderState* dS, uint32_t rare_stride) {
    if (!rare_stride) return nullptr;
    return (char*)ctx->rare_scratch.p + (size_t)(dS - (const FhRenderState*)ctx->state.p) * FH_RARE_BLOCKS * rare_stride;
}
static void tiles_by_groups(fhip_ctx* ctx, const RenderSetup& R, FhRenderState* dS, hipStream_t st) {
    const int gg = blocks_for(ctx, R.lds_tiles_group, 8);
    KaTiles ka = {dS, 0, 1, R.group_regs, R.group_choices, (uint32_t)gg, (ctx->probe ? 1u : 0u) | 2u | 4u | 8u, 0, 0};
    (void)launch_asm(ctx, st, FH_ASM_TILES, (uint32_t)gg, &ka, sizeof(ka), R.lds_tiles_group);
    const uint32_t blocks = R.S.qcap[0], root_words = (R.S.troot_choices + 15) / 16, group_words = (R.group_choices + 15) / 16;
    if (R.S.top_chain && R.S.n_top > 64u * FH_CHAIN_SEG) FH_KLAUNCH(k_tchain3d_chunks, dim3(WAVE, blocks), dim3(WAVE), 0, st, dS);
    else if (R.S.top_chain) FH_KLAUNCH(k_tchain3d, dim3(WAVE, blocks), dim3(WAVE), 0, st, dS);
    else FH_KLAUNCH(k_ttop3d, dim3(blocks), dim3(WAVE), 0, st, dS);
    if (R.classify_only || !root_words) FH_KLAUNCH(k_tmark3d, dim3(blocks), dim3(WAVE), 0, st, dS);
    if (R.classify_only) return;
    if (root_words) FH_KLAUNCH(k_tscatter3d, dim3(root_words + 1, blocks), dim3(WAVE), 0, st, dS, group_words, root_words);
    KaPrune1 kp = {dS, 0, 1, R.S.troot_choices, 2};
    if (!R.prune2) { (void)launch_asm(ctx, st, FH_ASM_PRUNE1, blocks * 64, &kp, sizeof(kp)); return; }
    hipEvent_t ea = nullptr, eb = nullptr;
    if (ctx->profiling) { (void)hipEventCreate(&ea); (void)hipEventCreate(&eb); (void)hipEventRecord(ea, st); }
    FH_KLAUNCH(k_prune2, dim3(blocks * FH_P2_PER_SLOT), dim3(FH_P2_WPB * FH_P2_WPC * 64), R.lds_prune2, st, dS, 0u, 1u, root_words,
                       (const uint2*)R.d_links, (const uint2*)R.d_ctab, 2u, R.S.troot_len, R.S.troot_choices, R.p2_cap_kept,
                       (const uint32_t*)(R.d_ctab + std::max<uint32_t>(R.S.troot_choices, 1)), R.n_chain);
    size_t kp_bytes = sizeof(kp);
    void* extra[] = {HIP_LAUNCH_PARAM_BUFFER_POINTER, &kp, HIP_LAUNCH_PARAM_BUFFER_SIZE, &kp_bytes, HIP_LAUNCH_PARAM_END};
    (void)hipModuleLaunchKernel(ctx->asm_fn[FH_ASM_PRUNE1], blocks * 64, 1, 1, WAVE, 1, 1, 0, st, nullptr, extra);
    if (ctx->profiling) { (void)hipEventRecord(eb, st); ctx->asm_events.push_back({FH_ASM_PRUNE1, {ea, eb}}); }
}
static void tiles_asm(fhip_ctx* ctx, const RenderSetup& R, const LevelPlan& L, FhRenderState* dS, int level, FrameStreams& fs) {
    const int gs = blocks_for(ctx, R.lds_tiles_small, 8), gb = blocks_big(ctx, R, R.lds_tiles_big, 8);
    const int K_TILES = R.asm_tiles_t ? FH_ASM_TILES_T : FH_ASM_TILES;
    auto big_stream = [&] { return L.fork_big ? fs.s[SIDE] : fs.on(); };
    KaTiles ka = {dS, (uint32_t)level, 0, SMALL_REGS, SMALL_CHOICES, (uint32_t)gs, (ctx->probe ? 1u : 0u) | (L.exp ? 2u : 0u), 0, 0};
    if (L.fork_big) { (void)hipEventRecord(ctx->ev_rest_fork, fs.on()); (void)hipStreamWaitEvent(fs.s[SIDE], ctx->ev_rest_fork, 0); }
    if (L.v32) {
        ka.n_waves = (uint32_t)(ctx->n_cu * 32);
        (void)launch_asm(ctx, fs.on(), R.asm_tiles_t ? FH_ASM_TILES_V32_T : FH_ASM_TILES_V32, ka.n_waves, &ka, sizeof(ka));
    } else if (L.small_lds)
        (void)launch_asm(ctx, fs.on(), K_TILES, (uint32_t)gs, &ka, sizeof(ka), R.lds_tiles_small);
    ka.big = 1;
    if (L.exp) ka.flags |= ((R.S.P.max_choices + 15) / 16) << 16;
    if (L.rare) return;
    if (L.v64) {
        ka.max_regs = V64_REGS; ka.max_choices = V64_CHOICES;
        ka.n_waves = L.per_slab ? 128u : (uint32_t)(ctx->n_cu * 8);
        if (L.both_lists) ka.flags |= 16u;
        (void)launch_asm(ctx, big_stream(), R.asm_tiles_t ? FH_ASM_TILES_V64_T : FH_ASM_TILES_V64, ka.n_waves, &ka, sizeof(ka));
        (void)hop(fs, L.rest_on, ctx->ev_l1);
        ka.flags &= ~16u;
        ka.skip_regs = V64_REGS; ka.skip_choices = V64_CHOICES;
    }
    if (L.mid) {
        const int gm = blocks_for(ctx, R.lds_tiles_mid, 8);
        ka.max_regs = MID_REGS; ka.max_choices = MID_CHOICES; ka.n_waves = (uint32_t)gm;
        (void)launch_asm(ctx, big_stream(), K_TILES, (uint32_t)gm, &ka, sizeof(ka), R.lds_tiles_mid);
        ka.skip_regs = MID_REGS; ka.skip_choices = MID_CHOICES;
    }
    ka.max_regs = R.S.P.max_regs; ka.max_choices = R.S.P.max_choices; ka.n_waves = (uint32_t)gb;
    if (L.rest) (void)launch_asm(ctx, big_stream(), K_TILES, (uint32_t)gb, &ka, sizeof(ka), R.lds_tiles_big);
    if (L.fork_big) { (void)hipEventRecord(ctx->ev_rest_join, fs.s[SIDE]); (void)hipStreamWaitEvent(fs.on(), ctx->ev_rest_join, 0); }
    if (L.exp) {
        KaPrune1 kp = {dS, (uint32_t)level, 0, SMALL_CHOICES, 0};
        const uint32_t bound = R.S.qcap[level] * 64;
        if (level > 0) (void)launch_asm(ctx, fs.on(), FH_ASM_PRUNE1, bound, &kp, sizeof(kp));
        kp.big = 1; kp.max_choices = R.S.P.max_choices;
        (void)launch_asm(ctx, fs.on(), FH_ASM_PRUNE1, bound, &kp, sizeof(kp));
    }
}
static void tiles_hip(fhip_ctx* ctx, const RenderSetup& R, FhRenderState* dS, int level, hipStream_t st) {
    const int gs = blocks_for(ctx, R.lds_tiles_small, 8), gb = blocks_big(ctx, R, R.lds_tiles_big, 8);
    if (level > 0 && R.full) FH_KLAUNCH((k_teval3d<true, false>), dim3(gs), dim3(WAVE), R.lds_tiles_small, st, dS, level);
    else if (level > 0) FH_KLAUNCH((k_teval3d<false, false>), dim3(gs), dim3(WAVE), R.lds_tiles_small, st, dS, level);
    if (R.full) FH_KLAUNCH((k_teval3d<true, true>), dim3(gb), dim3(WAVE), R.lds_tiles_big, st, dS, level);
    else FH_KLAUNCH((k_teval3d<false, true>), dim3(gb), dim3(WAVE), R.lds_tiles_big, st, dS, level);
}
static void launch_tiles_mono(fhip_ctx* ctx, const RenderSetup& R, FhRenderState* dS, int level, bool is3d, hipStream_t st) {
    const int gs = blocks_for(ctx, R.lds_tiles_small, 8), gb = blocks_big(ctx, R, R.lds_tiles_big, 8);
    launch(ctx, st, FHIP_K_TILES, [&] {
        if (is3d) { if (R.full) FH_LAUNCH_TILES(true, true, true, gb, R.lds_tiles_big); else FH_LAUNCH_TILES(true, false, true, gb, R.lds_tiles_big); }
        else { if (R.full) FH_LAUNCH_TILES(false, true, true, gb, R.lds_tiles_big); else FH_LAUNCH_TILES(false, false, true, gb, R.lds_tiles_big); }
    });
    if (level > 0)
        launch(ctx, st, FHIP_K_TILES, [&] {
            if (is3d) { if (R.full) FH_LAUNCH_TILES(true, true, false, gs, R.lds_tiles_small); else FH_LAUNCH_TILES(true, false, false, gs, R.lds_tiles_small); }
            else { if (R.full) FH_LAUNCH_TILES(false, true, false, gs, R.lds_tiles_small); else FH_LAUNCH_TILES(false, false, false, gs, R.lds_tiles_small); }
        });
}
static void launch_tiles(fhip_ctx* ctx, const RenderSetup& R, const LevelPlan& L, FhRenderState* dS, int level, bool is3d, FrameStreams& fs) {
    if (L.path == LevelPlan::MONO) return launch_tiles_mono(ctx, R, dS, level, is3d, fs.on());
    const int gp = ctx->n_cu * 8;
    launch(ctx, fs.on(), FHIP_K_TILES, [&] {
        if (is3d) FH_KLAUNCH(k_tsetup3d, dim3(gp), dim3(WAVE), 0, fs.on(), dS, level);
        else FH_KLAUNCH(k_tsetup2d, dim3(gp), dim3(WAVE), 0, fs.on(), dS, level);
    });
    launch(ctx, fs.on(), FHIP_K_TILES, [&] {
        if (L.path == LevelPlan::GROUPS) tiles_by_groups(ctx, R, dS, fs.on());
        else if (L.path == LevelPlan::ASM) tiles_asm(ctx, R, L, dS, level, fs);
        else tiles_hip(ctx, R, dS, level, fs.on());
    });
    const bool last = level + 1 == (int)R.S.P.n_levels;
    const int gpush = last ? ctx->n_cu * L.push_mul : gp;
    launch(ctx, fs.on(), FHIP_K_TILES, [&] {
        const uint32_t rb = L.rare ? FH_RARE_BLOCKS : 0u;
        if (is3d) FH_KLAUNCH(k_tpush3d, dim3(gpush + rb, last ? 1 : 17), dim3(WAVE), 0, fs.on(), dS, level, rb, rare_file(ctx, dS, L.rare_stride), L.rare_stride);
        else {
            if (!R.classify_only) FH_KLAUNCH(k_tpush2d, dim3(gpush), dim3(WAVE), 0, fs.on(), dS, level);
            const uint32_t slots_max = R.S.qcap[level] * ((level == 0 && R.groups) ? R.S.n_tgroups : 1u);
            FH_KLAUNCH(k_tfill2d, dim3(64, slots_max), dim3(256), 0, fs.on(), dS, level);
        }
    });
}

static fhip_status render2d_frame(fhip_ctx* ctx, const fhip_tape* tape, const fhip_render2d_config* cfg, float* out,
                                  int out_is_device) {
    if (ctx->is_cancelled()) return fail(ctx, FHIP_ERR_CANCELLED, "cancelled");
    RenderSetup R;
    memset(&R.S, 0, sizeof(R.S));
    FhRender& P = R.S.P;
    P.width = cfg->width; P.height = cfg->height; P.depth = 0; P.z = cfg->z; P.pixel_perfect = cfg->pixel_perfect ? 1 : 0;
    fhip_status st = bind_inputs(ctx, tape, cfg->axis_slots, cfg->var_keys, cfg->var_values, cfg->n_vars, P);
    if (st) return st;
    const uint32_t size[2] = {cfg->width, cfg->height};
    float s2w[9], m3[9];
    const float ident[9] = {1, 0, 0, 0, 1, 0, 0, 0, 1};
    fhip_screen_to_world(size, 2, s2w);
    mat_product(cfg->world_to_model ? cfg->world_to_model : ident, s2w, 3, m3);
    const float m4[16] = {m3[0], m3[1], 0, m3[2], m3[3], m3[4], 0, m3[5], 0, 0, 1, 0, m3[6], m3[7], 0, m3[8]};
    memcpy(P.mat, m4, sizeof(m4));
    std::vector<uint32_t> ts = cfg->tile_sizes ? trim_tiles(cfg->tile_sizes, cfg->n_tile_sizes, std::max(cfg->width, cfg->height))
                                               : trim_tiles(HIP_TILES_2D, 2, std::max(cfg->width, cfg->height));
    std::vector<uint32_t> tags;
    {
        std::vector<uint32_t> out;
        for (size_t i = 0; i < ts.size(); i++) {
            if (i) {
                uint32_t a = ts[i - 1];
                const uint32_t b = ts[i];
                if (a <= b || a % b) return fail(ctx, FHIP_ERR_UNSUPPORTED, "bad tile size list");
                while (a / b > 8) {
                    uint32_t c = 0;
                    for (uint32_t k = 8; k >= 2 && !c; k--) if (a % k == 0 && (a / k) % b == 0 && a / k > b) c = a / k;
                    if (!c) break;
                    out.push_back(c); tags.push_back((uint32_t)i);
                    a = c;
                }
            }
            out.push_back(ts[i]); tags.push_back((uint32_t)i);
        }
        if (out.size() > FH_MAX_LEVELS) return fail(ctx, FHIP_ERR_UNSUPPORTED, "1..8 tile levels supported");
        ts = out;
    }
    const size_t npix = (size_t)cfg->width * cfg->height;
    float* d_out = out;
    if (!out_is_device) { HIP_TRY(ctx, ctx->tmp_out.ensure(npix * 4)); d_out = (float*)ctx->tmp_out.p; }
    const TapeFacts facts = tape_facts(tape);
    auto pass = [&](RenderSetup& Q, const std::vector<uint32_t>& tiles, const std::vector<uint32_t>& tg) -> fhip_status {
        for (size_t i = 0; i < FH_MAX_LEVELS; i++) Q.S.P.tag[i] = i < tg.size() ? tg[i] : (uint32_t)i;
        fhip_status ps = prepare(ctx, tape, facts, false, tiles, PartSpec{}, Q);
        if (ps) return ps;
        Q.S.image2d = d_out;
        FhRenderState* dS = (FhRenderState*)ctx->state.p;
        const FrameClear no_clear[3] = {};
        FrameStreams fs = frame_streams(ctx);
        hipStream_t const st = fs.on();
        ps = upload_frame(ctx, st, tape, Q, no_clear);
        if (ps) return ps;
        for (uint32_t l = 0; l < Q.S.P.n_levels; l++) {
            if (ctx->is_cancelled()) return fail(ctx, FHIP_ERR_CANCELLED, "cancelled");
            launch_tiles(ctx, Q, plan_level(Q, schedule_inputs(ctx, out_is_device), (int)l, false, 0u, CALLER, CALLER), dS, (int)l, false, fs);
        }
        if (Q.classify_only) return FHIP_OK;
        launch(ctx, st, FHIP_K_POINTS, [&] {
            if (Q.full) FH_KLAUNCH((k_pixels2d<32, true>), dim3(ctx->n_cu * 8), dim3(WAVE), 0, st, dS);
            else FH_KLAUNCH((k_pixels2d<32, false>), dim3(ctx->n_cu * 16), dim3(WAVE), 0, st, dS);
        });
        if (Q.S.P.max_regs > 32)
            launch(ctx, st, FHIP_K_POINTS, [&] {
                const int g = blocks_big(ctx, Q, Q.lds_points_big, 16);
                if (Q.full) FH_KLAUNCH((k_pixels2d<0, true>), dim3(g), dim3(WAVE), Q.lds_points_big, st, dS);
                else FH_KLAUNCH((k_pixels2d<0, false>), dim3(g), dim3(WAVE), Q.lds_points_big, st, dS);
            });
        if (ctx->host_flags) FH_KLAUNCH(k_latch_arena, dim3(1), dim3(1), 0, st, dS, 1u, ctx->host_flags);
        return FHIP_OK;
    };
    const bool small_ok = ts.size() == 2 && tags.size() == 2 && ts[1] >= 8 && ts[0] / ts[1] <= 8 && ctx->opt.root32_max > 0 && linked_root_tape(facts, plan_inputs(ctx)) &&
                          (uint64_t)((P.width + ts[1] - 1) / ts[1]) * ((P.height + ts[1] - 1) / ts[1]) <= 2048u &&
                          (uint64_t)((P.width + ts[0] - 1) / ts[0]) * ((P.height + ts[0] - 1) / ts[0]) <= 64u;
    if (small_ok) {
        RenderSetup A = R;
        A.one_level_64 = true;
        st = pass(A, std::vector<uint32_t>{ts[1]}, std::vector<uint32_t>{1u});
        if (st) return st;
        if (!P.pixel_perfect) {
            RenderSetup B = R;
            B.one_level_64 = true; B.classify_only = true;
            st = pass(B, std::vector<uint32_t>{ts[0]}, std::vector<uint32_t>{0u});
            if (st) return st;
        }
    } else {
        st = pass(R, ts, tags);
        if (st) return st;
    }
    HIP_TRY(ctx, hipGetLastError());
    HIP_TRY(ctx, hipEventRecord(ctx->ev_done, ctx->stream));
    ctx->ev_done_valid = true;
    if (!out_is_device) {
        HIP_TRY(ctx, hipMemcpyAsync(out, d_out, npix * 4, hipMemcpyDeviceToHost, ctx->stream));
        return finish_render(ctx);
    }
    return FHIP_OK;
}

static void slab_begin(fhip_ctx* ctx, const RenderSetup& R, const FrameSchedule& F, FhRenderState* dS, int k, hipStream_t st) {
    const FhRender& P = R.S.P;
    const uint32_t pre = R.S.pre_levels, n_groups = R.groups_per_slab, n32 = ((P.width + 31) / 32) * ((P.height + 31) / 32);
    launch(ctx, st, FHIP_K_OTHER, [&] {
        const bool pyr3 = P.n_levels == 3 && P.tiles[2] == 8 && P.tiles[1] == 32 && P.tiles[0] == 128 && n32 <= 1024;
        const bool rebuild = k != F.slab_first;
        const bool pyr2 = P.n_levels == 2 && P.tiles[1] == 8 && P.tiles[0] == 32 && pre == 1;
        if (rebuild && pyr2) { FH_KLAUNCH(k_slab_begin2, dim3(n32 + F.reset_blocks), dim3(256), 0, st, dS, n32, F.table_words, (uint32_t)k, n_groups); return; }
        if (rebuild && pyr3 && pre == 2) { FH_KLAUNCH(k_slab_begin3, dim3(n32 + F.reset_blocks), dim3(256), 0, st, dS, n32, F.table_words, (uint32_t)k, n_groups); return; }
        FH_KLAUNCH(k_reset_slab, dim3(F.reset_blocks * 4), dim3(WAVE), 0, st, dS, F.table_words, (uint32_t)k, n_groups, (pyr3 && rebuild) ? 1u : 0u);
        if (rebuild && pyr3) FH_KLAUNCH(k_minpyramid3, dim3(n32), dim3(256), 0, st, dS);
        else if (rebuild) FH_KLAUNCH(k_minpyramid, dim3(P.roots_x * P.roots_y), dim3(256), 0, st, dS);
    });
}
static fhip_status tile_step(fhip_ctx* ctx, const RenderSetup& R, const FrameSchedule& F, FrameStreams& fs, FhRenderState* dS, int k, int idx) {
    fs.cur = F.tiles;
    if (F.pipe && idx >= (int)F.NC) HIP_TRY(ctx, hipStreamWaitEvent(fs.on(), ctx->ev_leaves[idx - (int)F.NC], 0));
    slab_begin(ctx, R, F, dS, k, fs.on());
    for (uint32_t l = R.S.pre_levels; l < R.S.P.n_levels; l++) launch_tiles(ctx, R, F.level[l], dS, (int)l, true, fs);
    if (F.pipe) HIP_TRY(ctx, hipEventRecord(ctx->ev_tiles[idx], fs.on()));
    fs.cur = CALLER;
    return FHIP_OK;
}
static void classify_work(fhip_ctx* ctx, const RenderSetup& R, const FrameSchedule& F, FhRenderState* dS, hipStream_t st) {
    const uint32_t class_blocks = (R.n_footprints + FH_CLASSIFY_FP - 1) / FH_CLASSIFY_FP;
    if (F.by_list && F.rare && R.S.P.max_regs > R.S.leaf_asm_regs)
        launch(ctx, st, FHIP_K_OTHER, [&] { FH_KLAUNCH(k_classify3d, dim3(FH_RARE_BLOCKS), dim3(WAVE), 0, st, dS, 1, 0u, rare_file(ctx, dS, F.rare_stride), F.rare_stride); });
    else if (!F.by_list) launch(ctx, st, FHIP_K_OTHER, [&] {
        FH_KLAUNCH(k_classify3d, dim3(class_blocks + (F.rare ? FH_RARE_BLOCKS : 0u)), dim3(R.S.P.slab / 8 > 16 ? 256 : WAVE), 0, st, dS, R.asm_points ? 1 : 0, class_blocks,
                   rare_file(ctx, dS, F.rare_stride), F.rare_stride);
    });
    if (R.S.P.max_regs > R.S.leaf_asm_regs && !F.rare)
        launch(ctx, st, FHIP_K_POINTS, [&] {
            const int g = blocks_big(ctx, R, R.lds_points_big, 16);
            if (R.full) FH_KLAUNCH((k_leaves3d<2, 0, 1, true>), dim3(g), dim3(WAVE), R.lds_points_big, st, dS);
            else FH_KLAUNCH((k_leaves3d<2, 0, 1, false>), dim3(g), dim3(WAVE), R.lds_points_big, st, dS);
        });
}
static void leaf_work(fhip_ctx* ctx, const RenderSetup& R, const FrameSchedule& F, FhRenderState* dS, uint32_t sk, hipStream_t st) {
    launch(ctx, st, FHIP_K_POINTS, [&] {
        if (F.leaf_walk == FrameSchedule::HIP_LEAVES) {
            const int per_cu = R.full ? 8 : 16;
            if (R.full) { FH_KLAUNCH((k_leaves3d<0, 16, 4, true>), dim3(ctx->n_cu * per_cu), dim3(WAVE), 0, st, dS); FH_KLAUNCH((k_leaves3d<1, 32, 2, true>), dim3(ctx->n_cu * per_cu), dim3(WAVE), 0, st, dS); }
            else { FH_KLAUNCH((k_leaves3d<0, 16, 4, false>), dim3(ctx->n_cu * per_cu), dim3(WAVE), 0, st, dS); FH_KLAUNCH((k_leaves3d<1, 32, 2, false>), dim3(ctx->n_cu * per_cu), dim3(WAVE), 0, st, dS); }
            return;
        }
        const int which = R.asm_points_t ? FH_ASM_COLUMNS_T : FH_ASM_COLUMNS;
        const uint32_t layers = R.S.P.slab / 8;
        const void* const slab_table = sk == 0 ? (const void*)R.S.leaf_table : (const void*)((const FhLeafRef*)ctx->leaf_table_b.p + (size_t)(sk - 1) * R.S.leaf_cap);
        const void* const slab_leaves = sk == 0 ? (const void*)R.S.leaves : (const void*)((const FhLeaf*)ctx->leaves_b.p + (size_t)(sk - 1) * R.S.leaf_cap);
        KaColumns ka = {dS, 0u, R.col_slots, R.col_depmask, R.col_flags, {0, 0}, slab_table, R.n_footprints, layers};
        if (F.leaf_walk == FrameSchedule::BY_LIST) {
            ka.flags |= (3u << 20) | (6u << 24); ka.pad[0] = F.list_waves; ka.table = slab_leaves; ka.nfpl = R.S.leaf_cap;
            (void)launch_asm(ctx, st, which, F.list_waves, &ka, sizeof(ka));
        } else if (F.leaf_walk == FrameSchedule::BY_COLUMNS) {
            ka.flags |= (1u << 20) | (F.g << 24);
            (void)launch_asm(ctx, st, which, (R.n_footprints + 63) / 64 * 64, &ka, sizeof(ka), 0, (layers + (1u << F.g) - 1) >> F.g);
        } else {
            const uint32_t n_blocks = (R.n_footprints + 3) / 4;
            ka.pad[0] = n_blocks > 1 ? (uint32_t)(((uint64_t)1 << 32) / n_blocks) : 0u;
            (void)launch_asm(ctx, st, which, n_blocks, &ka, sizeof(ka), 0, layers);
        }
    });
}
static void normals_work(fhip_ctx* ctx, const RenderSetup& R, const FrameSchedule& F, FhRenderState* dS, int k, hipStream_t st) {
    const uint32_t z_lo = (uint32_t)k * R.S.P.slab, z_hi = z_lo + R.S.P.slab;
    launch(ctx, st, FHIP_K_NORMALS, [&] {
        const int gs = blocks_for(ctx, R.lds_normals_small, 8), gb = blocks_big(ctx, R, R.lds_normals_big, 8);
        const int which = R.asm_points_t ? FH_ASM_NORMALS_T : FH_ASM_NORMALS;
        if (F.by_list) {
            if (F.rare && R.S.P.max_regs > R.S.norm_asm_regs)
                FH_KLAUNCH(k_hits3d, dim3(FH_RARE_BLOCKS), dim3(WAVE), 0, st, dS, z_lo, z_hi, R.hit_bucket_cap, 0u, rare_file(ctx, dS, F.rare_stride), F.rare_stride);
            KaNormals kn = {dS, F.list_waves, R.col_slots, z_lo, z_hi, R.hit_bucket_cap, 1u};
            (void)launch_asm(ctx, st, which, kn.n_waves, &kn, sizeof(kn));
        }
        else if (R.asm_normals) {
            const uint32_t hb = std::min<uint32_t>(R.n_footprints, (uint32_t)ctx->n_cu * 64);
            FH_KLAUNCH(k_hits3d, dim3(hb + (F.rare ? FH_RARE_BLOCKS : 0u)), dim3(WAVE), 0, st, dS, z_lo, z_hi, R.hit_bucket_cap, hb, rare_file(ctx, dS, F.rare_stride), F.rare_stride);
            KaNormals kn = {dS, std::max<uint32_t>((uint32_t)(ctx->n_cu * 8) / FH_HIT_BUCKETS, 1u) * FH_HIT_BUCKETS, R.col_slots, z_lo, z_hi, R.hit_bucket_cap, 0};
            (void)launch_asm(ctx, st, which, kn.n_waves, &kn, sizeof(kn));
        }
        else if (R.full) FH_KLAUNCH((k_normals3d<true, false>), dim3(gs), dim3(WAVE), R.lds_normals_small, st, dS, z_lo, z_hi);
        else FH_KLAUNCH((k_normals3d<false, false>), dim3(gs), dim3(WAVE), R.lds_normals_small, st, dS, z_lo, z_hi);
        if (R.S.P.max_regs > R.S.norm_asm_regs && !(F.rare && R.asm_normals)) {
            if (R.full) FH_KLAUNCH((k_normals3d<true, true>), dim3(gb), dim3(WAVE), R.lds_normals_big, st, dS, z_lo, z_hi);
            else FH_KLAUNCH((k_normals3d<false, true>), dim3(gb), dim3(WAVE), R.lds_normals_big, st, dS, z_lo, z_hi);
        }
    });
}
static fhip_status coarse_levels(fhip_ctx* ctx, const RenderSetup& R, const FrameSchedule& F, FrameStreams& fs, FhRenderState* dS) {
    const uint32_t pre = R.S.pre_levels;
    FhFork fork{};
    fork.n = F.NC; fork.mark = F.coarse ? 1u : 0u;
    fork.leaves = (FhLeaf*)ctx->leaves_b.p; fork.leaf_table = (FhLeafRef*)ctx->leaf_table_b.p; fork.fp_lists = (uint32_t*)ctx->fp_lists_b.p;
    fork.leaf_cap = (size_t)R.S.leaf_cap; fork.n_footprints = (size_t)R.n_footprints; fork.hit_words = R.hit_words;
    const bool forked_here = F.coarse && R.zrep;
    if (F.coarse) {
        launch_tiles(ctx, R, F.level[0], dS, 0, true, fs);
        if (pre > 1) {
            HIP_TRY(ctx, hop(fs, F.l1_flags, ctx->ev_l0));
            if (R.zrep) launch(ctx, fs.on(), FHIP_K_OTHER, [&] { FH_KLAUNCH(k_tape_flags, dim3(ctx->n_cu * 4), dim3(WAVE), 0, fs.on(), dS, 1, R.col_depmask, 0, FhFork{}); });
            HIP_TRY(ctx, hop(fs, F.l1, ctx->ev_l0));
            launch_tiles(ctx, R, F.level[1], dS, 1, true, fs);
        }
        HIP_TRY(ctx, hop(fs, F.fork_on, pre > 1 ? ctx->ev_l1 : ctx->ev_l0));
        if (R.zrep) launch(ctx, fs.on(), FHIP_K_OTHER, [&] { FH_KLAUNCH(k_tape_flags, dim3(ctx->n_cu * 8 + 1), dim3(WAVE), 0, fs.on(), dS, (int)pre, R.col_depmask, 1, fork); });
        if (!F.pipe && !forked_here) launch(ctx, fs.on(), FHIP_K_OTHER, [&] { FH_KLAUNCH(k_mark_frame, dim3(1), dim3(1), 0, fs.on(), dS); });
    }
    if (F.pipe) {
        if (!forked_here) FH_KLAUNCH(k_fork_state, dim3(1), dim3(1), 0, fs.on(), dS, fork);
        HIP_TRY(ctx, hipEventRecord(ctx->ev_fork, fs.on()));
        if (F.fork_to_side) HIP_TRY(ctx, hipStreamWaitEvent(fs.s[SIDE], ctx->ev_fork, 0));
    }
    if (F.ev_pre) HIP_TRY(ctx, hop(fs, CALLER, ctx->ev_pre));
    fs.cur = CALLER;
    if (F.fork_to_tail) HIP_TRY(ctx, hipStreamWaitEvent(fs.s[TAIL], ctx->ev_fork, 0));
    return FHIP_OK;
}
static fhip_status render_slabs(fhip_ctx* ctx, const RenderSetup& R, const FrameSchedule& F, FrameStreams& fs, FhRenderState* dS0) {
    auto slab_state = [&](int idx) { return dS0 + (F.pipe ? (uint32_t)idx % F.NC : 0u); };
    for (int idx = 0; F.tiles_first && idx < F.n_rendered; idx++) { const fhip_status st = tile_step(ctx, R, F, fs, slab_state(idx), F.slab_first - idx, idx); if (st) return st; }
    for (int idx = 0; idx < F.n_rendered; idx++) {
        if (ctx->is_cancelled()) return fail(ctx, FHIP_ERR_CANCELLED, "cancelled");
        const int k = F.slab_first - idx;
        FhRenderState* const dS = slab_state(idx);
        if (!F.tiles_first) { const fhip_status st = tile_step(ctx, R, F, fs, dS, k, idx); if (st) return st; }
        if (F.pipe) HIP_TRY(ctx, hipStreamWaitEvent(fs.s[F.leaf], ctx->ev_tiles[idx], 0));
        if (F.aux_edge) HIP_TRY(ctx, hipStreamWaitEvent(fs.s[F.lists], ctx->ev_tiles[idx], 0));
        classify_work(ctx, R, F, dS, fs.s[F.lists]);
        leaf_work(ctx, R, F, dS, (uint32_t)(dS - dS0), fs.s[F.leaf]);
        if (F.aux_edge) { HIP_TRY(ctx, hipEventRecord(ctx->ev_aux[idx], fs.s[F.leaf])); HIP_TRY(ctx, hipStreamWaitEvent(fs.s[F.normals], ctx->ev_aux[idx], 0)); }
        if (F.normals_on) normals_work(ctx, R, F, dS, k, fs.s[F.normals]);
        if (F.pipe) HIP_TRY(ctx, hipEventRecord(ctx->ev_leaves[idx], fs.s[F.normals]));
    }
    if (F.aux_edge && F.n_rendered > 0) HIP_TRY(ctx, hipStreamWaitEvent(fs.s[CALLER], ctx->ev_leaves[F.n_rendered - 1], 0));
    return FHIP_OK;
}

static fhip_status render3d_frame(fhip_ctx* ctx, const fhip_tape* tape, const fhip_render3d_config* cfg, void* out,
                                  int out_is_device, const PartSpec& part) {
    if (ctx->is_cancelled()) return fail(ctx, FHIP_ERR_CANCELLED, "cancelled");
    if (ctx->opt.stats & 2) g_spans.start();
    (void)hipSetDevice(ctx->device);
    RenderSetup R;
    memset(&R.S, 0, sizeof(R.S));
    FhRender& P = R.S.P;
    P.width = cfg->width; P.height = cfg->height; P.depth = cfg->depth; P.z = 0; P.pixel_perfect = 0;
    fhip_status st = bind_inputs(ctx, tape, cfg->axis_slots, cfg->var_keys, cfg->var_values, cfg->n_vars, P);
    if (st) return st;
    const uint32_t size[3] = {cfg->width, cfg->height, cfg->depth};
    float s2w[16];
    const float ident[16] = {1, 0, 0, 0, 0, 1, 0, 0, 0, 0, 1, 0, 0, 0, 0, 1};
    fhip_screen_to_world(size, 3, s2w);
    mat_product(cfg->world_to_model ? cfg->world_to_model : ident, s2w, 4, P.mat);
    const TapeFacts facts = tape_facts(tape);
    const PlanInputs pin = plan_inputs(ctx);
    column_facts(P, facts, pin, R);
    const TileChoice tiles = choose_tiles_3d(cfg->tile_sizes, cfg->n_tile_sizes, size, part.n_shards * part.nx * part.ny, part.nz, R.column_inv, pin.root32_max, pin.no_zrep,
                                             linked_root_tape(facts, pin));
    if (!tiles.valid) return fail(ctx, FHIP_ERR_UNSUPPORTED, "bad tile size list");
    if (tiles.substituted) ctx->substituted_tiles++;
    ScheduleInputs in = schedule_inputs(ctx, out_is_device);
    in.huge = (size_t)std::max<uint32_t>(tape->t.n_regs, 1) * WAVE * 16 > FH_LDS_MAX || tiles_lds(std::max<uint32_t>(tape->t.n_regs, 1), tape->t.n_choices, 64) > FH_LDS_MAX;
    in.whole = part.n_shards == 1 && part.nx * part.ny * part.nz == 1;
    if (frame_pipelined(in)) {
        for (uint32_t i = 0; i < ctx->extra_sets; i++) std::swap(static_cast<FrameBufs&>(*ctx), ctx->others[i]);
        in.frames_queued = ctx->extra_sets > 0 && ctx->others[0].ev_done_valid && hipEventQuery(ctx->others[0].ev_done) == hipErrorNotReady;
        (void)hipGetLastError();
    }
    FH_SPAN(0);
    st = prepare(ctx, tape, facts, true, tiles.ts, part, R);
    if (st) return st;
    FH_SPAN(1);
    in.pre_turn = ctx->pre_turn;
    if (ctx->host_flags) { in.rare_seen = ctx->host_flags[2]; in.last_leaves = ctx->host_flags[3]; }
    const FrameSchedule F = schedule_frame(R, in);
    if (F.takes_turn) ctx->pre_turn++;
    if (F.rare) { HIP_TRY(ctx, ctx->rare_scratch.ensure((size_t)F.rare_stride * FH_RARE_BLOCKS * 4)); ctx->rare_frames++; }
    R.S.leaf_list = F.by_list ? 1u : 0u; ctx->forked = F.pipe ? F.NC : 0;
    FrameStreams fs = frame_streams(ctx, F.root);
    if (F.fpipe && ctx->ev_done_valid) HIP_TRY(ctx, hipStreamWaitEvent(fs.on(), ctx->ev_done, 0));
    const size_t npix = (size_t)cfg->width * cfg->height;
    FhGeometryPixel* d_out = (FhGeometryPixel*)out;
    if (!out_is_device) { HIP_TRY(ctx, ctx->tmp_out.ensure(npix * sizeof(FhGeometryPixel))); d_out = (FhGeometryPixel*)ctx->tmp_out.p; }
    FhRenderState* const dS0 = (FhRenderState*)ctx->state.p;
    const FrameClear clear3[3] = {{ctx->zbuf.p, npix * 8, 0u}, {ctx->normals.p, npix * 12, 0u}, {ctx->mind.p, R.mind_words * 4, 0u}};
    st = upload_frame(ctx, fs.on(), tape, R, clear3);
    if (st) return st;
    FH_SPAN(2);
    st = coarse_levels(ctx, R, F, fs, dS0);
    if (st) return st;
    FH_SPAN(3);
    st = render_slabs(ctx, R, F, fs, dS0);
    if (st) return st;
    FH_SPAN(4);
    launch(ctx, ctx->stream, FHIP_K_OTHER, [&] { FH_KLAUNCH(k_finish3d, dim3(ctx->n_cu * 16), dim3(WAVE), 0, ctx->stream, dS0, d_out, std::max<uint32_t>(ctx->forked, 1u), (uint32_t*)ctx->sticky.p, ctx->host_flags); });
    HIP_TRY(ctx, hipGetLastError());
    if (ctx->launch_failed) { ctx->launch_failed = false; return FHIP_ERR_HIP; }
    ctx->async_pending = out_is_device != 0;
    HIP_TRY(ctx, hipEventRecord(ctx->ev_done, ctx->stream));
    ctx->ev_done_valid = true;
    if (ctx->opt.stats & 2) { g_spans.mark(5); g_spans.frame(); }
    if (!out_is_device) {
        HIP_TRY(ctx, hipMemcpyAsync(out, d_out, npix * sizeof(FhGeometryPixel), hipMemcpyDeviceToHost, ctx->stream));
        return finish_render(ctx);
    }
    return FHIP_OK;
}
static bool lanes_possible(fhip_ctx* ctx, int out_is_device) {
    if (ctx->opt.frame_lanes < 2 || ctx->is_lane || !out_is_device || ctx->profiling || ctx->probe || (ctx->opt.stats & 1)) return false;
    if (!ctx->ev_last_valid) return false;
    const hipError_t q = hipEventQuery(ctx->ev_last);
    (void)hipGetLastError();
    return q == hipErrorNotReady;
}
static void lane_tune_release(fhip_ctx* ctx);
static void lanes_release(fhip_ctx* ctx, bool keep_measurements) {
    if (!keep_measurements) lane_tune_release(ctx);
    for (fhip_ctx* L : ctx->lanes) {
        hipStream_t const s = L->lane_stream_owned ? L->stream : nullptr;
        if (L->lane_done) (void)hipEventDestroy(L->lane_done);
        if (L->lane_copied) (void)hipEventDestroy(L->lane_copied);
        L->lane_img.release();
        fhip_ctx_destroy(L);
        if (s) (void)hipStreamDestroy(s);
    }
    ctx->lanes.clear();
}
static fhip_status run_on_lane_(fhip_ctx* ctx, uint32_t max_lanes, size_t bytes, void* out, const std::function<fhip_status(fhip_ctx*, void*)>& render) {
    const uint32_t K = std::min((uint32_t)std::min(ctx->opt.frame_lanes, 8), max_lanes);
    if (ctx->opt.lanes_fail) return fail(ctx, FHIP_ERR_HIP, "frame lanes: failure provoked (option lanes_fail)");
    while (ctx->lanes.size() < K) {
        hipStream_t const mine[3] = {ctx->stream_pre, ctx->stream3, ctx->stream2};
        const size_t k = ctx->lanes.size();
        hipStream_t s = k < 3 ? mine[k] : nullptr;
        const bool owned = !s;
        if (owned) HIP_TRY(ctx, hipStreamCreateWithFlags(&s, hipStreamNonBlocking));
        fhip_ctx* L = nullptr;
        const fhip_status st = fhip_ctx_create(ctx->device, (void*)s, &L);
        if (st) { if (owned) (void)hipStreamDestroy(s); return fail(ctx, st, "frame lanes: no child context"); }
        L->lane_stream_owned = owned;
        L->opt = ctx->opt;
        L->opt.no_pipeline = 1;
        L->opt.frame_lanes = 0;
        apply_options(L);
        L->is_lane = true;
        (void)hipEventCreateWithFlags(&L->lane_done, hipEventDisableTiming);
        (void)hipEventCreateWithFlags(&L->lane_copied, hipEventDisableTiming);
        ctx->lanes.push_back(L);
    }
    fhip_ctx* const L = ctx->lanes[ctx->lane_next++ % K];
    L->cancel_src = &ctx->cancelled;
    L->watch.store(ctx->watch.load(std::memory_order_relaxed), std::memory_order_relaxed);
    HIP_TRY(ctx, L->lane_img.ensure(bytes));
    if (L->lane_copied_valid) HIP_TRY(ctx, hipStreamWaitEvent(L->stream, L->lane_copied, 0));
    const fhip_status st = render(L, L->lane_img.p);
    if (st) { ctx->err = L->err; return st; }
    HIP_TRY(ctx, hipEventRecord(L->lane_done, L->stream));
    HIP_TRY(ctx, hipStreamWaitEvent(ctx->stream, L->lane_done, 0));
    HIP_TRY(ctx, hipMemcpyAsync(out, L->lane_img.p, bytes, hipMemcpyDeviceToDevice, ctx->stream));
    HIP_TRY(ctx, hipEventRecord(L->lane_copied, ctx->stream));
    L->lane_copied_valid = true;
    ctx->lane_frames++;
    if (ctx->tune_cur < 0) ctx->lane_frames_wanted++;
    return FHIP_OK;
}
static const fhip_status FHIP_LANE_FALLBACK = (fhip_status)1000;
static fhip_status run_on_lane(fhip_ctx* ctx, uint32_t max_lanes, size_t bytes, void* out, const std::function<fhip_status(fhip_ctx*, void*)>& render) {
    ctx->last_hip_error = 0;
    for (fhip_ctx* L : ctx->lanes) if (L) L->last_hip_error = 0;
    const fhip_status st = run_on_lane_(ctx, max_lanes, bytes, out, render);
    if (st != FHIP_ERR_HIP) return st;
    bool resources = ctx->opt.lanes_fail != 0 || ctx->last_hip_error == (int)hipErrorOutOfMemory || ctx->err.rfind("frame lanes:", 0) == 0;
    for (fhip_ctx* L : ctx->lanes) if (L && L->last_hip_error == (int)hipErrorOutOfMemory) resources = true;
    if (!resources) return st;
    if (ctx->mesh_leaves.cap) {
        (void)hipDeviceSynchronize();
        ctx->mesh_leaves.release();
    }
    fprintf(stderr, "fidget-hip: frame lanes given up for this context (%s); frames keep to the stage pipeline\n", ctx->err.c_str());
    (void)hipGetLastError();
    (void)hipStreamSynchronize(ctx->stream);
    ctx->opt.frame_lanes = 0;
    lanes_release(ctx);
    ctx->err.clear();
    return FHIP_LANE_FALLBACK;
}
static constexpr uint32_t TUNE_SKIP = 4, TUNE_WIN = 8;
static uint32_t tune_lanes(const fhip_ctx* ctx) { return (uint32_t)std::min(std::max(ctx->opt.frame_lanes, 2), 8); }
static void lane_tune_release(fhip_ctx* ctx) {
    for (auto& t : ctx->lane_tune)
        for (hipEvent_t& e : t.ev) if (e) { (void)hipEventDestroy(e); e = nullptr; }
    ctx->lane_tune.clear();
    ctx->tune_last_key = 0;
    ctx->tune_cur = -1;
}
static bool lane_mode(fhip_ctx* ctx, const fhip_tape* tape, const fhip_render3d_config* cfg, int out_is_device, const PartSpec& part) {
    ctx->tune_cur = -1;
    const bool whole = part.n_shards == 1 && part.nx * part.ny * part.nz == 1;
    const bool possible = lanes_possible(ctx, out_is_device) && ctx->use_pipeline && ctx->frame_pipeline;
    const bool prior = ctx->use_asm && !ctx->opt.no_columns_t && !tape_asm_ok(tape->t);
    if (!possible) { ctx->tune_last_key = 0; return false; }
    uint64_t key = (tape->parent_serial ? tape->parent_serial : tape->serial) * 0x9E3779B97F4A7C15ull;
    key ^= ((uint64_t)cfg->width << 42) ^ ((uint64_t)cfg->height << 21) ^ (uint64_t)cfg->depth;
    key ^= (((uint64_t)part.shard * 64 + part.n_shards) * 0xD6E8FEB86659FD93ull) ^ ((((uint64_t)part.ix * 16 + part.iy) * 16 + part.iz) * 4096 + (part.nx * 16 + part.ny) * 16 + part.nz) * 0xA24BAED4963EE407ull;
    key |= 1;
    int at = -1;
    for (size_t i = 0; i < ctx->lane_tune.size(); i++) if (ctx->lane_tune[i].key == key) at = (int)i;
    if (at < 0) {
        if (ctx->lane_tune.size() < 32) { ctx->lane_tune.emplace_back(); at = (int)ctx->lane_tune.size() - 1; }
        else {
            at = 0;
            for (size_t i = 1; i < ctx->lane_tune.size(); i++) if (ctx->lane_tune[i].used < ctx->lane_tune[at].used) at = (int)i;
            for (hipEvent_t& e : ctx->lane_tune[at].ev) if (e) { (void)hipEventDestroy(e); e = nullptr; }
            ctx->lane_tune[at] = fhip_ctx::LaneTune();
        }
        ctx->lane_tune[at].key = key;
    }
    fhip_ctx::LaneTune& T = ctx->lane_tune[at];
    T.used = ++ctx->tune_clock;
    if (T.phase == 4) { ctx->tune_last_key = key; return T.lanes; }
    if (ctx->tune_last_key != key) {
        ctx->tune_last_key = key;
        if (T.phase < 3) { T.n = 0; return prior; }
    }
    if (T.phase == 3) {
        const hipError_t q = hipEventQuery(T.ev[5]);
        (void)hipGetLastError();
        if (q != hipSuccess) return false;
        bool ok = true;
        for (int w = 0; w < 3; w++) {
            float t = 0.0f;
            ok = ok && hipEventElapsedTime(&t, T.ev[2 * w], T.ev[2 * w + 1]) == hipSuccess && t > 0.0f;
            T.ms[w] = t / (w == 1 ? 2 * tune_lanes(ctx) : TUNE_WIN);
        }
        (void)hipGetLastError();
        T.lanes = ok ? T.ms[1] < 0.97f * std::min(T.ms[0], T.ms[2]) : prior;
        T.phase = 4;
        if (!T.lanes && ctx->lane_frames_wanted == 0) {
            bool others = false;
            for (const fhip_ctx::LaneTune& o : ctx->lane_tune) others = others || (&o != &T && (o.phase != 4 || o.lanes));
            if (!others) lanes_release(ctx, true);
        }
        return T.lanes;
    }
    ctx->tune_cur = at;
    return T.phase == 1;
}
static fhip_status frame_queued(fhip_ctx* ctx, int out_is_device) {
    if (!out_is_device || ctx->is_lane || ctx->opt.frame_lanes < 2) return FHIP_OK;
    if (!ctx->ev_last) HIP_TRY(ctx, hipEventCreateWithFlags(&ctx->ev_last, hipEventDisableTiming));
    HIP_TRY(ctx, hipEventRecord(ctx->ev_last, ctx->stream));
    ctx->ev_last_valid = true;
    if (ctx->tune_cur >= 0) {
        fhip_ctx::LaneTune& T = ctx->lane_tune[(size_t)ctx->tune_cur];
        ctx->tune_cur = -1;
        T.n++;
        const uint32_t K = tune_lanes(ctx);
        const uint32_t skip = T.phase == 1 ? K : TUNE_SKIP, win = T.phase == 1 ? 2 * K : TUNE_WIN, tail = T.phase == 1 ? K : 0u;
        if (T.n == skip || T.n == skip + win) {
            hipEvent_t& e = T.ev[2 * T.phase + (T.n == skip ? 0 : 1)];
            if (!e) HIP_TRY(ctx, hipEventCreate(&e));
            HIP_TRY(ctx, hipEventRecord(e, ctx->stream));
        }
        if (T.n == skip + win + tail) { T.phase++; T.n = 0; }
    }
    return FHIP_OK;
}
static fhip_status render3d_part(fhip_ctx* ctx, const fhip_tape* tape, const fhip_render3d_config* cfg, void* out,
                                 int out_is_device, const PartSpec& part) {
    (void)hipSetDevice(ctx->device);
    std::shared_ptr<const fhip_tape> bound;
    fhip_render3d_config bcfg;
    if (tape->t.n_vars > FH_MAX_INPUTS) {
        const fhip_status bs = bound_tape(ctx, tape, cfg->axis_slots, cfg->var_keys, cfg->var_values, cfg->n_vars, bound);
        if (bs) return bs;
        tape = bound.get();
        bcfg = *cfg; bcfg.axis_slots = BOUND_AXES; bcfg.var_keys = nullptr; bcfg.var_values = nullptr; bcfg.n_vars = 0;
        cfg = &bcfg;
    }
    fhip_status st = lane_mode(ctx, tape, cfg, out_is_device, part)
        ? run_on_lane(ctx, 8, (size_t)cfg->width * cfg->height * sizeof(FhGeometryPixel), out,
                      [&](fhip_ctx* L, void* img) { return render3d_frame(L, tape, cfg, img, 1, part); })
        : render3d_frame(ctx, tape, cfg, out, out_is_device, part);
    if (st == FHIP_LANE_FALLBACK) st = render3d_frame(ctx, tape, cfg, out, out_is_device, part);
    if (st) ctx->tune_cur = -1;
    return st ? st : frame_queued(ctx, out_is_device);
}
fhip_status fhip_render2d(fhip_ctx* ctx, const fhip_tape* tape, const fhip_render2d_config* cfg, float* out, int out_is_device) {
    (void)hipSetDevice(ctx->device);
    std::shared_ptr<const fhip_tape> bound;
    fhip_render2d_config bcfg;
    if (tape->t.n_vars > FH_MAX_INPUTS) {
        const fhip_status bs = bound_tape(ctx, tape, cfg->axis_slots, cfg->var_keys, cfg->var_values, cfg->n_vars, bound);
        if (bs) return bs;
        tape = bound.get();
        bcfg = *cfg; bcfg.axis_slots = BOUND_AXES; bcfg.var_keys = nullptr; bcfg.var_values = nullptr; bcfg.n_vars = 0;
        cfg = &bcfg;
    }
    ctx->tune_cur = -1;
    ctx->tune_last_key = 0;
    fhip_status st = lanes_possible(ctx, out_is_device)
        ? run_on_lane(ctx, 3, (size_t)cfg->width * cfg->height * 4, out, [&](fhip_ctx* L, void* img) { return render2d_frame(L, tape, cfg, (float*)img, 1); })
        : render2d_frame(ctx, tape, cfg, out, out_is_device);
    if (st == FHIP_LANE_FALLBACK) st = render2d_frame(ctx, tape, cfg, out, out_is_device);
    return st ? st : frame_queued(ctx, out_is_device);
}
fhip_status fhip_render3d(fhip_ctx* ctx, const fhip_tape* tape, const fhip_render3d_config* cfg, void* out,
                          int out_is_device) {
    return render3d_part(ctx, tape, cfg, out, out_is_device, PartSpec{});
}
fhip_status fhip_render3d_shard(fhip_ctx* ctx, const fhip_tape* tape, const fhip_render3d_config* cfg, void* out,
                                int out_is_device, uint32_t shard, uint32_t n_shards) {
    if (n_shards == 0 || shard >= n_shards) return fail(ctx, FHIP_ERR_UNSUPPORTED, "bad shard");
    PartSpec p;
    p.shard = shard; p.n_shards = n_shards;
    return render3d_part(ctx, tape, cfg, out, out_is_device, p);
}
fhip_status fhip_render3d_block(fhip_ctx* ctx, const fhip_tape* tape, const fhip_render3d_config* cfg, void* out,
                                int out_is_device, uint32_t index, const uint32_t split[3]) {
    if (!split || !split[0] || !split[1] || !split[2] || index >= split[0] * split[1] * split[2]) return fail(ctx, FHIP_ERR_UNSUPPORTED, "bad block");
    PartSpec p;
    p.nx = split[0]; p.ny = split[1]; p.nz = split[2];
    p.ix = index % p.nx; p.iy = (index / p.nx) % p.ny; p.iz = index / (p.nx * p.ny);
    return render3d_part(ctx, tape, cfg, out, out_is_device, p);
}
fhip_status fhip_merge_depth(fhip_ctx* ctx, void* front, const void* back, uint64_t n_pixels, uint32_t image_depth) {
    if (!n_pixels) return FHIP_OK;
    (void)hipSetDevice(ctx->device);
    FH_KLAUNCH(k_merge_depth, dim3((unsigned)std::min<uint64_t>((n_pixels + 255) / 256, 65535)), dim3(256), 0, ctx->stream,
                       (FhGeometryPixel*)front, (const FhGeometryPixel*)back, (size_t)n_pixels, image_depth);
    HIP_TRY(ctx, hipGetLastError());
    return FHIP_OK;
}
```

fidget_amd/csrc/capi_tapes.hpp:

```cpp
static fhip_status finish_tape(fhip_ctx* ctx, fh::SsaProgram& prog, fhip_tape** out) {
    std::string err;
    fhip_tape* t = new fhip_tape();
    if (!fh::allocate(prog, t->t, err)) { delete t; return fail(ctx, FHIP_ERR_UNSUPPORTED, err); }
    if (t->t.n_vars > FH_MAX_TAPE_VARS) { delete t; return fail(ctx, FHIP_ERR_UNSUPPORTED, "more than 2^20 input variables"); }
    const size_t min_ops = getenv("FHIP_GROUPS_MIN_OPS") ? (size_t)atol(getenv("FHIP_GROUPS_MIN_OPS")) : 1024;
    const uint32_t min_terms = getenv("FHIP_GROUPS_MIN_TERMS") ? (uint32_t)atol(getenv("FHIP_GROUPS_MIN_TERMS")) : 32;
    const uint32_t want_groups = (uint32_t)std::min<long>(FH_MAX_GROUPS, std::max<long>(2, getenv("FHIP_GROUPS") ? atol(getenv("FHIP_GROUPS")) : 32));
    if (t->t.ops.size() >= min_ops && !getenv("FHIP_NO_GROUPS")) {
        std::vector<fh::SsaProgram> gp;
        const int op = fh::split_root(prog, want_groups, min_terms, gp);
        if (op >= 0) {
            t->groups.resize(gp.size());
            bool ok = true;
            for (size_t g = 0; g < gp.size() && ok; g++) ok = fh::allocate(gp[g], t->groups[g], err);
            if (ok) t->group_op = op; else t->groups.clear();
        }
        if (fh::plan_terms(prog, want_groups, min_terms, 16, t->plan)) {
            t->tgroups.resize(t->plan.groups.size());
            bool ok = true;
            for (size_t g = 0; g < t->tgroups.size() && ok; g++) ok = fh::allocate(t->plan.groups[g], t->tgroups[g], err);
            if (!ok) t->tgroups.clear();
            t->plan.groups.clear();
        }
    }
    *out = t;
    return FHIP_OK;
}
uint32_t fhip_tape_group_count(const fhip_tape* tape) { return (uint32_t)tape->groups.size(); }
int fhip_tape_group_op(const fhip_tape* tape) { return tape->group_op; }
fhip_status fhip_tape_group(fhip_ctx* ctx, const fhip_tape* tape, uint32_t g, fhip_tape** out) {
    if (g >= tape->groups.size()) return fail(ctx, FHIP_ERR_BAD_TAPE, "no such tape group");
    fhip_tape* t = new fhip_tape();
    t->t = tape->groups[g];
    *out = t;
    return FHIP_OK;
}
fhip_status fhip_tape_term_group(fhip_ctx* ctx, const fhip_tape* tape, uint32_t g, fhip_tape** out) {
    if (g >= tape->tgroups.size()) return fail(ctx, FHIP_ERR_BAD_TAPE, "no such term group");
    fhip_tape* t = new fhip_tape();
    t->t = tape->tgroups[g];
    *out = t;
    return FHIP_OK;
}
uint32_t fhip_tape_term_tree(const fhip_tape* tape, uint32_t* words, uint32_t cap_ops) {
    const uint32_t n = (uint32_t)std::min<size_t>(tape->plan.top.size(), cap_ops);
    for (uint32_t i = 0; i < n; i++) {
        const fh::TopOp& o = tape->plan.top[i];
        words[3 * i] = (uint32_t)o.op | ((uint32_t)o.out << 8) | ((uint32_t)o.a_kind << 16) | ((uint32_t)o.b_kind << 24);
        words[3 * i + 1] = o.a; words[3 * i + 2] = o.b;
    }
    return (uint32_t)tape->plan.top.size();
}
uint32_t fhip_tape_term_choice_src(const fhip_tape* tape, uint32_t* src, uint32_t cap) {
    const uint32_t n = (uint32_t)std::min<size_t>(tape->plan.choice_src.size(), cap);
    for (uint32_t i = 0; i < n; i++) src[i] = tape->plan.choice_src[i];
    return (uint32_t)tape->plan.choice_src.size();
}
uint32_t fhip_tape_term_plan(const fhip_tape* tape, uint32_t info[4]) {
    info[0] = tape->plan.n_terms; info[1] = (uint32_t)tape->plan.top.size(); info[2] = tape->plan.top_regs;
    info[3] = (uint32_t)tape->plan.choice_src.size();
    return (uint32_t)tape->tgroups.size();
}
static hipError_t launch_asm(fhip_ctx* ctx, hipStream_t st, int which, uint32_t waves, void* args, size_t bytes, size_t lds = 0, uint32_t grid_y = 1) {
    void* extra[] = {HIP_LAUNCH_PARAM_BUFFER_POINTER, args, HIP_LAUNCH_PARAM_BUFFER_SIZE, &bytes, HIP_LAUNCH_PARAM_END};
    hipEvent_t ea = nullptr, eb = nullptr;
    if (ctx->profiling) { (void)hipEventCreate(&ea); (void)hipEventCreate(&eb); (void)hipEventRecord(ea, st); }
    const hipError_t e = hipModuleLaunchKernel(ctx->asm_fn[which], waves, grid_y, 1, WAVE, 1, 1, (unsigned)lds, st, nullptr, extra);
    if (ctx->profiling) { (void)hipEventRecord(eb, st); ctx->asm_events.push_back({which, {ea, eb}}); }
    if (e != hipSuccess) {
        ctx->launch_failed = true;
        if (ctx->err.empty()) ctx->err = std::string("launch of ") + FH_ASM_NAMES[which] + ": " + hipGetErrorString(e);
    }
    return e;
}
static bool tape_tiles_t_ok(const fh::HostTape&) { return true; }
static std::vector<uint32_t> chain_table(const fhip_tape* tape, const std::vector<uint64_t>& cops) {
    std::vector<uint32_t> chain;
    if (tape->plan.chain && tape->plan.top.size() < 65536) {
        chain.assign(tape->plan.top.size(), 0xFFFFFFFFu);
        for (size_t q = 0; q < tape->plan.choice_src.size() && q < cops.size(); q++)
            if ((tape->plan.choice_src[q] >> 24) == 255 && (tape->plan.choice_src[q] & 0xFFFFFFu) < chain.size())
                chain[tape->plan.choice_src[q] & 0xFFFFFFu] = (uint32_t)q | ((uint32_t)((cops[q] >> 32) & 0xFFFFu) << 16);
        for (uint32_t c : chain) if (c == 0xFFFFFFFFu) { chain.clear(); break; }
    }
    return chain;
}

static uint32_t tape_class(const fh::HostTape& t) {
    uint32_t c = __atomic_load_n(&t.op_class, __ATOMIC_ACQUIRE);
    if (c) return c;
    c = 1;
    for (uint64_t w : t.ops) {
        const uint32_t op = FH_W_OP((uint32_t)w);
        if ((op >= FH_SIN && op <= FH_LN) || op == FH_RAND) c |= 2;
        if (op >= FH_SIN && op <= FH_LN) c |= 8;
        if (op >= FH_ADD_RR) {
            const int base = op >= FH_SUB_IR ? (int[]){1, 3, 4, 5, 6, 7}[op - FH_SUB_IR] : (int)((op - FH_ADD_RR) % 12);
            if (base == 4 || base == 6 || base == 7) c |= 2;
            if (base == 4 || base == 7) c |= 8;
            if (base == 7) c |= 4;
        }
    }
    __atomic_store_n(&t.op_class, c, __ATOMIC_RELEASE);
    return c;
}
static bool tape_has_mod(const fh::HostTape& t) { return (tape_class(t) & 4) != 0; }
static bool tape_asm_ok(const fh::HostTape& t) { return (tape_class(t) & 2) == 0; }
static bool tape_is_full(const fh::HostTape& t) { return (tape_class(t) & 8) != 0; }
static uint32_t tape_input_slots(const fhip_tape* tape) {
    uint32_t reads = tape->input_slots.load(std::memory_order_acquire);
    if (reads & 0x80000000u) {
        reads = 0;
        for (uint64_t w : tape->t.ops)
            if (FH_W_OP((uint32_t)w) == FH_INPUT) reads |= 1u << ((uint32_t)(w >> 32) & 31u);
        reads &= 0x7FFFFFFFu;
        tape->input_slots.store(reads, std::memory_order_release);
    }
    return reads;
}
static TapeFacts tape_facts(const fhip_tape* tape) {
    const fh::HostTape& t = tape->t;
    TapeFacts f;
    f.n_ops = t.ops.size(); f.n_regs = t.n_regs; f.n_choices = t.n_choices; f.n_outputs = t.n_outputs;
    f.asm_ok = tape_asm_ok(t); f.is_full = tape_is_full(t); f.has_mod = tape_has_mod(t); f.tiles_t_ok = tape_tiles_t_ok(t);
    f.input_slots = tape_input_slots(tape);
    f.n_groups = (uint32_t)std::min<size_t>(tape->tgroups.size(), FH_MAX_GROUPS);
    for (uint32_t g = 0; g < f.n_groups; g++) f.group[g] = {(uint32_t)tape->tgroups[g].ops.size(), tape->tgroups[g].n_regs, tape->tgroups[g].n_choices};
    f.n_terms = tape->plan.n_terms; f.n_top = (uint32_t)tape->plan.top.size(); f.chain = tape->plan.chain;
    return f;
}

static fhip_status tape_to_device(fhip_ctx* ctx, const fhip_tape* t) {
    std::lock_guard<std::mutex> guard(t->upload_lock);
    (void)hipSetDevice(ctx->device);
    if (t->device >= 0 && t->device != ctx->device) return fail(ctx, FHIP_ERR_UNSUPPORTED, "this tape's device copies belong to another device: build the tape per device");
    if (t->d_ops) return FHIP_OK;
    t->device = ctx->device;
    size_t bytes = (t->t.ops.size() + 16) * 8;
    uint64_t* d = nullptr;
    HIP_TRY(ctx, hipMalloc((void**)&d, bytes));
    HIP_TRY(ctx, hipMemset(d, 0, bytes));
    HIP_TRY(ctx, hipMemcpy(d, t->t.ops.data(), t->t.ops.size() * 8, hipMemcpyHostToDevice));
    t->d_ops = d;
    return FHIP_OK;
}
fhip_status fhip_tape_from_bytecode(fhip_ctx* ctx, const uint32_t* words, size_t n_words, fhip_tape** out) {
    fh::SsaProgram prog;
    std::string err;
    if (!fh::from_bytecode(words, n_words, prog, err)) return fail(ctx, FHIP_ERR_BAD_TAPE, err);
    return finish_tape(ctx, prog, out);
}
fhip_status fhip_tape_from_graph(fhip_ctx* ctx, const fhip_graph* g, const uint32_t* roots, uint32_t n_roots,
                                 fhip_tape** out) {
    fh::SsaProgram prog;
    std::string err;
    std::vector<fh::NodeId> r(roots, roots + n_roots);
    if (!fh::flatten(g->g, r, prog, err)) return fail(ctx, FHIP_ERR_BAD_TAPE, err);
    return finish_tape(ctx, prog, out);
}
void fhip_tape_free(fhip_tape* t) {
    if (!t) return;
    if (t->d_ops) (void)hipFree(t->d_ops);
    if (t->d_top) (void)hipFree(t->d_top);
    if (t->d_chsrc) (void)hipFree(t->d_chsrc);
    if (t->d_links) (void)hipFree(t->d_links);
    if (t->d_ctab) (void)hipFree(t->d_ctab);
    delete t;
}
uint32_t fhip_tape_len(const fhip_tape* t) { return (uint32_t)t->t.ops.size(); }
uint32_t fhip_tape_choice_count(const fhip_tape* t) { return t->t.n_choices; }
uint32_t fhip_tape_reg_count(const fhip_tape* t) { return t->t.n_regs; }
uint32_t fhip_tape_var_count(const fhip_tape* t) { return t->t.n_vars; }
uint32_t fhip_tape_output_count(const fhip_tape* t) { return t->t.n_outputs; }
fhip_status fhip_tape_reg_tape(const fhip_tape* t, uint32_t n_regs, uint32_t* reg_ops, uint32_t cap_ops, uint32_t* words, uint32_t cap_words,
                               uint32_t info[4]) {
    fh::RegTapeOut rt;
    std::string err;
    for (int i = 0; i < 4; i++) info[i] = 0;
    if (!fh::reg_tape(t->t, n_regs, rt, err)) return FHIP_ERR_BAD_TAPE;
    info[0] = (uint32_t)rt.ops.size(); info[1] = rt.slot_count;
    if (reg_ops)
        for (size_t i = 0; i < rt.ops.size() && i < cap_ops; i++) {
            const fh::RegOp& o = rt.ops[rt.ops.size() - 1 - i];
            reg_ops[4 * i] = o.op; reg_ops[4 * i + 1] = o.out; reg_ops[4 * i + 2] = o.a;
            reg_ops[4 * i + 3] = fh_is_rr(o.op) ? (uint32_t)o.b : o.w;
        }
    std::vector<uint32_t> w;
    const bool ok = fh::reg_tape_bytecode(rt, n_regs, w, info[2], info[3]);
    if (!ok) return FHIP_ERR_UNSUPPORTED;
    if (words) for (size_t i = 0; i < w.size() && i < cap_words; i++) words[i] = w[i];
    return FHIP_OK;
}
uint32_t fhip_tape_ops(const fhip_tape* t, uint64_t* ops, uint32_t cap) {
    for (uint32_t i = 0; i < t->t.ops.size() && i < cap; i++) ops[i] = t->t.ops[i];
    return (uint32_t)t->t.ops.size();
}
int fhip_tape_axis_slot(const fhip_tape* t, int axis) { return (axis >= 0 && axis < 3) ? t->t.vars.axis[axis] : -1; }
int fhip_tape_var_slot(const fhip_tape* t, uint64_t index) { return t->t.vars.slot_of(3, index); }

fhip_status fhip_simplify(fhip_ctx* ctx, const fhip_tape* tape, const uint8_t* choices, uint32_t n_choices,
                          fhip_tape** child) {
    const fh::HostTape& p = tape->t;
    if (n_choices != p.n_choices) return fail(ctx, FHIP_ERR_BAD_CHOICE_SLICE, "choice slice length mismatch");
    fhip_tape* t = new fhip_tape();
    if (!simplify_host(p, choices, t->t)) { delete t; return fail(ctx, FHIP_ERR_BAD_CHOICE_SLICE, "Choice::Unknown in trace"); }
    *child = t;
    return FHIP_OK;
}
```

include/fidget_hip_debug.h:

```cpp
#ifndef FIDGET_HIP_DEBUG_H
#define FIDGET_HIP_DEBUG_H
#include "fidget_hip.h"
#ifdef __cplusplus
extern "C" {
#endif

fhip_status fhip_debug_stats(fhip_ctx* ctx, uint64_t out[64]);
fhip_status fhip_debug_leaf_stats(fhip_ctx* ctx, uint64_t out[8]);
uint32_t fhip_debug_tape_links(const fhip_tape* tape, uint64_t* out, uint32_t cap);
uint32_t fhip_debug_tape_chain(const fhip_tape* tape, uint32_t* out, uint32_t cap);
uint32_t fhip_debug_leaves(fhip_ctx* ctx, void* out, uint32_t cap);
fhip_status fhip_debug_probe(fhip_ctx* ctx, float* out);
uint64_t fhip_debug_lane_frames(const fhip_ctx* ctx);
uint64_t fhip_debug_rare_frames(const fhip_ctx* ctx);
int fhip_debug_lane_tune(const fhip_ctx* ctx, float ms[3], int* lanes);
fhip_status fhip_debug_trans_probe(fhip_ctx* ctx, uint32_t copy, uint32_t fn, uint32_t first, uint64_t n, uint64_t out[2]);
uint32_t fhip_debug_arena(fhip_ctx* ctx, uint32_t off, uint32_t n, uint64_t* out);
fhip_status fhip_debug_bound_tape(fhip_ctx* ctx, const fhip_tape* tape, const int32_t* axis_slots, const uint64_t* keys, const float* vals,
                                  uint32_t n, fhip_tape** out);
fhip_status fhip_debug_bench(fhip_ctx* ctx, const fhip_tape* tape, uint32_t n_waves, uint32_t reps, int variant,
                             double* ms);

fhip_status fhip_debug_ubench(fhip_ctx* ctx, uint32_t test, uint32_t iters, uint32_t n_waves, float* out);
fhip_status fhip_debug_math_sweep(fhip_ctx* ctx, int op, uint32_t first, uint32_t stride, uint64_t n, const float* ref, uint64_t out[4]);
uint32_t fhip_debug_groups(fhip_ctx* ctx, int kind, uint32_t index, void* out, uint32_t cap, uint32_t counts[2]);

void fhip_debug_walk_dual(const uint32_t* cells, uint64_t n_cells, const uint32_t* root, const float* verts, uint64_t n_verts, int parallel,
                          uint64_t counts[2], uint64_t* tris, float* verts_out);
fhip_status fhip_debug_stl_pack(fhip_ctx* ctx, const float* verts, uint64_t n_verts, const uint64_t* tris, uint64_t n_tris, void* out);

#ifdef __cplusplus
}
#endif
#endif
```

Baseline: 9.759 million Mvoxel/s.

## Record lane kernel launches and replay them as HIP graphs

Adds a launch-list recorder for frame-lane contexts. Kernel launches are captured into a list instead of being issued one by one, and each flush compares the list to the previous one and builds, replays or updates a HIP graph according to a streak policy, falling back to direct launches when the list changes too much. The goal is to cut per-kernel host launch overhead in the repeated render frames. The cost is graph build and compare work on the host, plus extra complexity; the probe option is also folded into a stats bit and lane tuning skips more frames.

```diff
diff --git a/fidget_amd/__init__.py b/fidget_amd/__init__.py
--- a/fidget_amd/__init__.py
+++ b/fidget_amd/__init__.py
@@ -10,7 +10,7 @@
 _HERE = os.path.dirname(os.path.abspath(__file__))
 _CSRC = os.path.join(_HERE, "csrc")
 LIB_PATH = os.environ.get("FHIP_LIB") or os.path.join(_CSRC, "libfidget_hip.so")
-_SOURCES = ["capi.hip", "capi_core.hpp", "capi_context.hpp", "capi_tapes.hpp", "capi_eval.hpp", "capi_render.hpp", "frame_plan.hpp", "frame_schedule.hpp", "capi_effects.hpp", "capi_mesh.hpp", "capi_debug.hpp", "capi_solve.hpp", "solve.hip", "solve_lm.hpp", "kernels.hip", "prune2.hip", "effects.hip", "mesh.hip", "mesh_qef.hpp", "mesh_collapse.hpp", "mesh_edges.hpp", "mesh_walk.hpp", "mesh_split.hpp", "mesh_vox.hpp", "mesh_cc.hpp", "mesh_edt.hpp", "edt.hip", "capi_edt.hpp", "mesh_vmesh.hpp", "vmesh.hip", "capi_vmesh.hpp", "contour/contour.hpp", "host_mesh.hpp", "dev_ops.hpp", "host_graph.hpp", "host_regtape.hpp", "render_state.h", "tape_format.h",
+_SOURCES = ["capi.hip", "capi_core.hpp", "capi_context.hpp", "capi_tapes.hpp", "capi_eval.hpp", "capi_render.hpp", "frame_plan.hpp", "launch_list.hpp", "frame_schedule.hpp", "capi_effects.hpp", "capi_mesh.hpp", "capi_debug.hpp", "capi_solve.hpp", "solve.hip", "solve_lm.hpp", "kernels.hip", "prune2.hip", "effects.hip", "mesh.hip", "mesh_qef.hpp", "mesh_collapse.hpp", "mesh_edges.hpp", "mesh_walk.hpp", "mesh_split.hpp", "mesh_vox.hpp", "mesh_cc.hpp", "mesh_edt.hpp", "edt.hip", "capi_edt.hpp", "mesh_vmesh.hpp", "vmesh.hip", "capi_vmesh.hpp", "contour/contour.hpp", "host_mesh.hpp", "dev_ops.hpp", "host_graph.hpp", "host_regtape.hpp", "render_state.h", "tape_format.h",
             "gen_interp.py", "gen_tiles.py", "gen_tilesv.py", "gen_normals.py", "gen_prune.py", "gen_ubench.py", "gen_trans.py", "trans_funcs.hip", "trans_libm.hpp", "offsets.cpp", "../../include/fidget_hip.h",
             "../../include/fidget_hip_debug.h"]
 
@@ -44,7 +44,7 @@
     "fhip_profile_enable", "fhip_profile_read", "fhip_profile_read_kernels", "fhip_render_counters", "fhip_graph_new", "fhip_graph_free",
     "fhip_graph_len", "fhip_graph_var", "fhip_graph_constant", "fhip_graph_unary", "fhip_graph_binary",
     "fhip_graph_from_text", "fhip_tape_from_graph", "fhip_tape_axis_slot", "fhip_tape_var_slot",
-    "fhip_screen_to_world", "fhip_debug_groups", "fhip_debug_ubench", "fhip_debug_math_sweep", "fhip_debug_stats", "fhip_debug_leaf_stats", "fhip_debug_tape_links", "fhip_debug_tape_chain", "fhip_debug_bench", "fhip_debug_leaves", "fhip_debug_arena", "fhip_debug_probe", "fhip_debug_trans_probe", "fhip_debug_bound_tape", "fhip_debug_lane_frames", "fhip_debug_rare_frames", "fhip_debug_lane_tune", "fhip_debug_walk_dual", "fhip_debug_stl_pack", "fhip_tape_group_count", "fhip_tape_group_op",
+    "fhip_screen_to_world", "fhip_debug_groups", "fhip_debug_ubench", "fhip_debug_math_sweep", "fhip_debug_stats", "fhip_debug_leaf_stats", "fhip_debug_tape_links", "fhip_debug_tape_chain", "fhip_debug_bench", "fhip_debug_leaves", "fhip_debug_arena", "fhip_debug_probe", "fhip_debug_trans_probe", "fhip_debug_bound_tape", "fhip_debug_lane_frames", "fhip_debug_lane_graph", "fhip_debug_rare_frames", "fhip_debug_lane_tune", "fhip_debug_walk_dual", "fhip_debug_stl_pack", "fhip_tape_group_count", "fhip_tape_group_op",
     "fhip_tape_group", "fhip_tape_term_plan", "fhip_tape_term_group", "fhip_tape_term_tree", "fhip_tape_term_choice_src",
 ]
 
@@ -186,6 +186,7 @@
             "fhip_debug_math_sweep": (i32, [vp, i32, u32, u32, u64, vp, vp]),
             "fhip_debug_trans_probe": (i32, [vp, u32, u32, u32, u64, vp]),
             "fhip_debug_lane_frames": (u64, [vp]),
+            "fhip_debug_lane_graph": (None, [vp, vp]),
             "fhip_debug_rare_frames": (u64, [vp]),
             "fhip_debug_lane_tune": (i32, [vp, vp, vp]),
             "fhip_debug_bound_tape": (i32, [vp, vp, vp, vp, vp, u32, C.POINTER(vp)]),
@@ -254,6 +255,11 @@
 
     def lane_frames(self):
         return int(lib().fhip_debug_lane_frames(self._h))
+
+    def lane_graph(self):
+        out = (C.c_uint64 * 4)()
+        lib().fhip_debug_lane_graph(self._h, out)
+        return {"built": int(out[0]), "replayed": int(out[1]), "updated": int(out[2]), "eager": int(out[3])}
 
     def rare_frames(self):
         return int(lib().fhip_debug_rare_frames(self._h))
diff --git a/fidget_amd/csrc/capi.hip b/fidget_amd/csrc/capi.hip
--- a/fidget_amd/csrc/capi.hip
+++ b/fidget_amd/csrc/capi.hip
@@ -24,6 +24,7 @@
 #include "solve.hip"
 #include "host_mesh.hpp"
 #include "frame_schedule.hpp"
+#include "launch_list.hpp"
 
 #include "capi_core.hpp"
 
diff --git a/fidget_amd/csrc/capi_core.hpp b/fidget_amd/csrc/capi_core.hpp
--- a/fidget_amd/csrc/capi_core.hpp
+++ b/fidget_amd/csrc/capi_core.hpp
@@ -63,11 +63,11 @@
                       \
     X(no_column_inv, 0) X(no_zrep, 0) X(root32_max, 4096) X(column_walk, 1) X(column_group, 2)                                                    \
                                                                                                  \
-    X(no_pipeline, 0) X(frame_lanes, 4) X(lanes_fail, 0) X(slab_layers, 4) X(arena_mb, 4096)  \
+    X(no_pipeline, 0) X(frame_lanes, 4) X(lane_graph, 1) X(lanes_fail, 0) X(slab_layers, 4) X(arena_mb, 4096)  \
           \
     X(mesh_device_assembly, 1) X(mesh_device_walk, 1) X(mesh_simplify_min_ops, 256) X(mesh_keep_device, 0)                      \
                                                                                                               \
-    X(probe, 0) X(stats, 0)
+    X(stats, 0)
 struct FhOptions {
 #define X(name, dflt) int name = dflt;
     FH_OPTION_LIST(X)
@@ -107,6 +107,22 @@
         ev_done = nullptr;
         bound_hold.reset();
     }
+};
+struct LaneGraphSlot {
+    fhll::LaunchList held;
+    bool have_held = false;
+    fhll::Policy policy;
+    hipGraph_t graph = nullptr;
+    hipGraphExec_t exec = nullptr;
+    std::vector<hipGraphNode_t> nodes;
+    std::vector<size_t> arg_bytes;
+};
+struct LaneRec {
+    bool on = false;
+    uint32_t flushes = 0;
+    fhll::LaunchList list;
+    std::vector<uint32_t> changed;
+    LaneGraphSlot slot[2];
 };
 struct fhip_ctx : FrameBufs {
     FhOptions opt;
@@ -184,13 +200,16 @@
     DevBuf lane_img;
     hipEvent_t lane_done = nullptr, lane_copied = nullptr;
     bool lane_copied_valid = false;
+    LaneRec rec;
+    fhip_ctx* lane_parent = nullptr;
+    uint64_t lane_graph_counts[4] = {0, 0, 0, 0};
 };
 
 #define FH_ARENA_START_MB 128
 static void apply_options(fhip_ctx* c) {
     c->use_asm = c->opt.no_asm == 0;
     c->use_split = c->opt.no_split == 0;
-    c->probe = c->opt.probe != 0;
+    c->probe = (c->opt.stats & 4) != 0;
     c->use_pipeline = c->opt.no_pipeline == 0;
     c->frame_pipeline = true;
     c->slab_contexts = 4;
@@ -277,6 +296,125 @@
     return true;
 }
 
+static void lane_graph_drop(LaneGraphSlot& s) {
+    if (s.exec) (void)hipGraphExecDestroy(s.exec);
+    if (s.graph) (void)hipGraphDestroy(s.graph);
+    s.exec = nullptr; s.graph = nullptr; s.nodes.clear();
+}
+static void lane_graph_release(fhip_ctx* ctx) {
+    for (LaneGraphSlot& s : ctx->rec.slot) { lane_graph_drop(s); s.held.clear(); s.have_held = false; s.policy = fhll::Policy(); }
+}
+static hipError_t lane_launch_direct(fhip_ctx* ctx, const fhll::LaunchList& l) {
+    hipError_t first = hipSuccess;
+    for (size_t i = 0; i < l.size(); i++) {
+        const fhll::Launch& k = l.v[i];
+        size_t bytes = k.arg_bytes;
+        void* extra[] = {HIP_LAUNCH_PARAM_BUFFER_POINTER, (void*)l.arg(i), HIP_LAUNCH_PARAM_BUFFER_SIZE, &bytes, HIP_LAUNCH_PARAM_END};
+        const hipError_t e = hipModuleLaunchKernel((hipFunction_t)k.fn, k.grid[0], k.grid[1], k.grid[2], k.block[0], k.block[1], k.block[2], k.lds, ctx->stream, nullptr, extra);
+        if (e != hipSuccess && first == hipSuccess) first = e;
+    }
+    if (first != hipSuccess) {
+        ctx->launch_failed = true;
+        ctx->last_hip_error = (int)first;
+        if (ctx->err.empty()) ctx->err = std::string("kernel launch: ") + hipGetErrorString(first);
+        (void)hipGetLastError();
+    }
+    return first;
+}
+static hipError_t lane_graph_node_params(LaneGraphSlot& s, size_t i, void** extra, hipKernelNodeParams& p) {
+    const fhll::Launch& k = s.held.v[i];
+    extra[0] = HIP_LAUNCH_PARAM_BUFFER_POINTER; extra[1] = (void*)s.held.arg(i); extra[2] = HIP_LAUNCH_PARAM_BUFFER_SIZE; extra[3] = &s.arg_bytes[i]; extra[4] = HIP_LAUNCH_PARAM_END;
+    memset(&p, 0, sizeof(p));
+    p.func = (void*)k.fn;
+    p.gridDim = dim3(k.grid[0], k.grid[1], k.grid[2]); p.blockDim = dim3(k.block[0], k.block[1], k.block[2]);
+    p.sharedMemBytes = k.lds; p.kernelParams = nullptr; p.extra = extra;
+    return hipSuccess;
+}
+static hipError_t lane_graph_build(LaneGraphSlot& s) {
+    lane_graph_drop(s);
+    s.arg_bytes.resize(s.held.size());
+    for (size_t i = 0; i < s.held.size(); i++) s.arg_bytes[i] = s.held.v[i].arg_bytes;
+    hipError_t e = hipGraphCreate(&s.graph, 0);
+    s.nodes.assign(s.held.size(), nullptr);
+    for (size_t i = 0; e == hipSuccess && i < s.held.size(); i++) {
+        void* extra[5];
+        hipKernelNodeParams p;
+        (void)lane_graph_node_params(s, i, extra, p);
+        e = hipGraphAddKernelNode(&s.nodes[i], s.graph, i ? &s.nodes[i - 1] : nullptr, i ? 1 : 0, &p);
+    }
+    if (e == hipSuccess) e = hipGraphInstantiate(&s.exec, s.graph, nullptr, nullptr, 0);
+    if (e != hipSuccess) lane_graph_drop(s);
+    return e;
+}
+static void lane_flush(fhip_ctx* ctx, bool direct = false) {
+    LaneRec& r = ctx->rec;
+    if (!r.on) return;
+    fhip_ctx* const parent = ctx->lane_parent ? ctx->lane_parent : ctx;
+    const bool counted = r.flushes == 0;
+    bool done = false;
+    if (!r.list.empty() && !direct && r.flushes < 2 && ctx->opt.lane_graph) {
+        LaneGraphSlot& s = r.slot[r.flushes];
+        const fhll::Diff d = s.have_held ? fhll::compare(s.held, r.list, r.changed) : fhll::REBUILD;
+        const fhll::Action a = fhll::decide(s.policy, s.exec != nullptr, s.have_held, d, r.changed.size(), r.list.size());
+        hipError_t e = hipSuccess;
+        switch (a) {
+        case fhll::DIRECT_DROP: lane_graph_drop(s); s.held = r.list; s.have_held = true; break;
+        case fhll::DIRECT: if (!s.exec) { s.held = r.list; s.have_held = true; } break;
+        case fhll::BUILD:
+            s.held = r.list; s.have_held = true;
+            e = lane_graph_build(s);
+            if (e == hipSuccess) { parent->lane_graph_counts[0]++; e = hipGraphLaunch(s.exec, ctx->stream); done = e == hipSuccess; if (done && counted) parent->lane_graph_counts[1]++; }
+            break;
+        case fhll::UPDATE:
+            for (size_t j = 0; e == hipSuccess && j < r.changed.size(); j++) {
+                const size_t i = r.changed[j];
+                memcpy(s.held.v[i].grid, r.list.v[i].grid, sizeof(s.held.v[i].grid));
+                if (s.held.v[i].arg_bytes) memcpy(s.held.arg(i), r.list.arg(i), s.held.v[i].arg_bytes);
+                void* extra[5];
+                hipKernelNodeParams p;
+                (void)lane_graph_node_params(s, i, extra, p);
+                e = hipGraphExecKernelNodeSetParams(s.exec, s.nodes[i], &p);
+            }
+            if (e == hipSuccess) { e = hipGraphLaunch(s.exec, ctx->stream); done = e == hipSuccess; if (done && counted) parent->lane_graph_counts[2]++; }
+            break;
+        case fhll::REPLAY:
+            e = hipGraphLaunch(s.exec, ctx->stream); done = e == hipSuccess; if (done && counted) parent->lane_graph_counts[1]++;
+            break;
+        }
+        if (e != hipSuccess) {
+            (void)hipGetLastError();
+            lane_graph_drop(s); s.have_held = false; s.policy = fhll::Policy();
+            if (parent->opt.lane_graph) fprintf(stderr, "fidget-hip: lane graphs given up for this context (%s); the lanes launch their kernels one by one\n", hipGetErrorString(e));
+            parent->opt.lane_graph = 0;
+            for (fhip_ctx* L : parent->lanes) if (L) L->opt.lane_graph = 0;
+            ctx->opt.lane_graph = 0;
+        }
+    }
+    if (!done && !r.list.empty()) { (void)lane_launch_direct(ctx, r.list); if (counted) parent->lane_graph_counts[3]++; }
+    if (!r.list.empty()) r.flushes++;
+    r.list.clear();
+}
+static void lane_rec_stop(fhip_ctx* ctx) {
+    if (!ctx->rec.on) return;
+    lane_flush(ctx, true);
+    ctx->rec.on = false;
+}
+static inline bool lane_record(fhip_ctx* ctx, hipStream_t st, hipFunction_t fn, dim3 g, dim3 b, size_t lds, const void* args, size_t bytes) {
+    if (!ctx->rec.on) return false;
+    if (st != ctx->stream || !fn) { lane_rec_stop(ctx); return false; }
+    ctx->rec.list.add((const void*)fn, g.x, g.y, g.z, b.x, b.y, b.z, (uint32_t)lds, args, bytes);
+    return true;
+}
+struct LaneRecScope {
+    fhip_ctx* ctx;
+    explicit LaneRecScope(fhip_ctx* c) : ctx(c) {
+        LaneRec& r = c->rec;
+        r.on = c->is_lane && c->opt.lane_graph != 0 && !c->profiling && !c->probe;
+        r.flushes = 0; r.list.clear();
+    }
+    ~LaneRecScope() { ctx->rec.on = false; ctx->rec.list.clear(); }
+};
+
 template <class T> struct FhKArgs;
 template <class... K> struct FhKArgs<void (*)(K...)> {
     template <class... A> static size_t pack(char* buf, A&&... a) {
@@ -308,11 +446,13 @@
     }
     hipError_t e;
     if (!fn) {
+        lane_rec_stop(ctx);
         hipLaunchKernelGGL(Kernel, g, b, lds, st, std::forward<A>(a)...);
         e = hipGetLastError();
     } else {
         alignas(16) char buf[FhKArgs<decltype(Kernel)>::bytes];
         size_t bytes = FhKArgs<decltype(Kernel)>::pack(buf, std::forward<A>(a)...);
+        if (lane_record(ctx, st, fn, g, b, lds, buf, bytes)) return;
         void* extra[] = {HIP_LAUNCH_PARAM_BUFFER_POINTER, buf, HIP_LAUNCH_PARAM_BUFFER_SIZE, &bytes, HIP_LAUNCH_PARAM_END};
         e = hipModuleLaunchKernel(fn, g.x, g.y, g.z, b.x, b.y, b.z, (unsigned)lds, st, nullptr, extra);
     }
diff --git a/fidget_amd/csrc/capi_debug.hpp b/fidget_amd/csrc/capi_debug.hpp
--- a/fidget_amd/csrc/capi_debug.hpp
+++ b/fidget_amd/csrc/capi_debug.hpp
@@ -145,6 +145,9 @@
     return n;
 }
 uint64_t fhip_debug_lane_frames(const fhip_ctx* ctx) { return ctx ? ctx->lane_frames : 0; }
+void fhip_debug_lane_graph(const fhip_ctx* ctx, uint64_t out[4]) {
+    for (int i = 0; i < 4; i++) out[i] = ctx ? ctx->lane_graph_counts[i] : 0;
+}
 int fhip_debug_lane_tune(const fhip_ctx* ctx, float ms[3], int* lanes) {
     if (!ctx) return -1;
     for (const auto& t : ctx->lane_tune)
diff --git a/fidget_amd/csrc/capi_render.hpp b/fidget_amd/csrc/capi_render.hpp
--- a/fidget_amd/csrc/capi_render.hpp
+++ b/fidget_amd/csrc/capi_render.hpp
@@ -233,7 +233,10 @@
         if (clear[k].p) most = std::max(most, clear[k].bytes);
     }
     const unsigned blocks = (unsigned)std::max<size_t>(8, std::min<size_t>((size_t)ctx->n_cu * 32, (most + 64 * 64 - 1) / (64 * 64)));
+    const bool recording = ctx->rec.on;
+    if (recording) { lane_flush(ctx); ctx->rec.on = false; }
     FH_KLAUNCH(k_frame_begin, dim3(blocks), dim3(WAVE), 0, st, fb);
+    ctx->rec.on = recording;
     HIP_TRY(ctx, hipGetLastError());
     HIP_TRY(ctx, hipEventRecord(sg.ev, st));
     sg.used = true;
@@ -293,7 +296,8 @@
                        (const uint32_t*)(R.d_ctab + std::max<uint32_t>(R.S.troot_choices, 1)), R.n_chain);
     size_t kp_bytes = sizeof(kp);
     void* extra[] = {HIP_LAUNCH_PARAM_BUFFER_POINTER, &kp, HIP_LAUNCH_PARAM_BUFFER_SIZE, &kp_bytes, HIP_LAUNCH_PARAM_END};
-    (void)hipModuleLaunchKernel(ctx->asm_fn[FH_ASM_PRUNE1], blocks * 64, 1, 1, WAVE, 1, 1, 0, st, nullptr, extra);
+    if (!lane_record(ctx, st, ctx->asm_fn[FH_ASM_PRUNE1], dim3(blocks * 64, 1, 1), dim3(WAVE, 1, 1), 0, &kp, kp_bytes))
+        (void)hipModuleLaunchKernel(ctx->asm_fn[FH_ASM_PRUNE1], blocks * 64, 1, 1, WAVE, 1, 1, 0, st, nullptr, extra);
     if (ctx->profiling) { (void)hipEventRecord(eb, st); ctx->asm_events.push_back({FH_ASM_PRUNE1, {ea, eb}}); }
 }
 static void tiles_asm(fhip_ctx* ctx, const RenderSetup& R, const LevelPlan& L, FhRenderState* dS, int level, FrameStreams& fs) {
@@ -423,7 +427,8 @@
     float* d_out = out;
     if (!out_is_device) { HIP_TRY(ctx, ctx->tmp_out.ensure(npix * 4)); d_out = (float*)ctx->tmp_out.p; }
     const TapeFacts facts = tape_facts(tape);
-    auto pass = [&](RenderSetup& Q, const std::vector<uint32_t>& tiles, const std::vector<uint32_t>& tg) -> fhip_status {
+    LaneRecScope lane_rec(ctx);
+    auto pass_launches = [&](RenderSetup& Q, const std::vector<uint32_t>& tiles, const std::vector<uint32_t>& tg) -> fhip_status {
         for (size_t i = 0; i < FH_MAX_LEVELS; i++) Q.S.P.tag[i] = i < tg.size() ? tg[i] : (uint32_t)i;
         fhip_status ps = prepare(ctx, tape, facts, false, tiles, PartSpec{}, Q);
         if (ps) return ps;
@@ -451,6 +456,11 @@
             });
         if (ctx->host_flags) FH_KLAUNCH(k_latch_arena, dim3(1), dim3(1), 0, st, dS, 1u, ctx->host_flags);
         return FHIP_OK;
+    };
+    auto pass = [&](RenderSetup& Q, const std::vector<uint32_t>& tiles, const std::vector<uint32_t>& tg) -> fhip_status {
+        const fhip_status ps = pass_launches(Q, tiles, tg);
+        if (ps == FHIP_OK) lane_flush(ctx);
+        return ps;
     };
     const bool small_ok = ts.size() == 2 && tags.size() == 2 && ts[1] >= 8 && ts[0] / ts[1] <= 8 && ctx->opt.root32_max > 0 && linked_root_tape(facts, plan_inputs(ctx)) &&
                           (uint64_t)((P.width + ts[1] - 1) / ts[1]) * ((P.height + ts[1] - 1) / ts[1]) <= 2048u &&
@@ -623,6 +633,7 @@
     if (ctx->is_cancelled()) return fail(ctx, FHIP_ERR_CANCELLED, "cancelled");
     if (ctx->opt.stats & 2) g_spans.start();
     (void)hipSetDevice(ctx->device);
+    LaneRecScope lane_rec(ctx);
     RenderSetup R;
     memset(&R.S, 0, sizeof(R.S));
     FhRender& P = R.S.P;
@@ -676,6 +687,7 @@
     if (st) return st;
     FH_SPAN(4);
     launch(ctx, ctx->stream, FHIP_K_OTHER, [&] { FH_KLAUNCH(k_finish3d, dim3(ctx->n_cu * 16), dim3(WAVE), 0, ctx->stream, dS0, d_out, std::max<uint32_t>(ctx->forked, 1u), (uint32_t*)ctx->sticky.p, ctx->host_flags); });
+    lane_flush(ctx);
     HIP_TRY(ctx, hipGetLastError());
     if (ctx->launch_failed) { ctx->launch_failed = false; return FHIP_ERR_HIP; }
     ctx->async_pending = out_is_device != 0;
@@ -703,6 +715,7 @@
         if (L->lane_done) (void)hipEventDestroy(L->lane_done);
         if (L->lane_copied) (void)hipEventDestroy(L->lane_copied);
         L->lane_img.release();
+        lane_graph_release(L);
         fhip_ctx_destroy(L);
         if (s) (void)hipStreamDestroy(s);
     }
@@ -726,6 +739,7 @@
         L->opt.frame_lanes = 0;
         apply_options(L);
         L->is_lane = true;
+        L->lane_parent = ctx;
         (void)hipEventCreateWithFlags(&L->lane_done, hipEventDisableTiming);
         (void)hipEventCreateWithFlags(&L->lane_copied, hipEventDisableTiming);
         ctx->lanes.push_back(L);
@@ -838,7 +852,7 @@
         ctx->tune_cur = -1;
         T.n++;
         const uint32_t K = tune_lanes(ctx);
-        const uint32_t skip = T.phase == 1 ? K : TUNE_SKIP, win = T.phase == 1 ? 2 * K : TUNE_WIN, tail = T.phase == 1 ? K : 0u;
+        const uint32_t skip = T.phase == 1 ? (ctx->opt.lane_graph ? 2 * K : K) : TUNE_SKIP, win = T.phase == 1 ? 2 * K : TUNE_WIN, tail = T.phase == 1 ? K : 0u;
         if (T.n == skip || T.n == skip + win) {
             hipEvent_t& e = T.ev[2 * T.phase + (T.n == skip ? 0 : 1)];
             if (!e) HIP_TRY(ctx, hipEventCreate(&e));
diff --git a/fidget_amd/csrc/capi_tapes.hpp b/fidget_amd/csrc/capi_tapes.hpp
--- a/fidget_amd/csrc/capi_tapes.hpp
+++ b/fidget_amd/csrc/capi_tapes.hpp
@@ -62,6 +62,7 @@
     return (uint32_t)tape->tgroups.size();
 }
 static hipError_t launch_asm(fhip_ctx* ctx, hipStream_t st, int which, uint32_t waves, void* args, size_t bytes, size_t lds = 0, uint32_t grid_y = 1) {
+    if (lane_record(ctx, st, ctx->asm_fn[which], dim3(waves, grid_y, 1), dim3(WAVE, 1, 1), lds, args, bytes)) return hipSuccess;
     void* extra[] = {HIP_LAUNCH_PARAM_BUFFER_POINTER, args, HIP_LAUNCH_PARAM_BUFFER_SIZE, &bytes, HIP_LAUNCH_PARAM_END};
     hipEvent_t ea = nullptr, eb = nullptr;
     if (ctx->profiling) { (void)hipEventCreate(&ea); (void)hipEventCreate(&eb); (void)hipEventRecord(ea, st); }
diff --git a/fidget_amd/csrc/launch_list.hpp b/fidget_amd/csrc/launch_list.hpp
--- /dev/null
+++ b/fidget_amd/csrc/launch_list.hpp
@@ -0,0 +1,83 @@
+#pragma once
+#include <stddef.h>
+#include <stdint.h>
+#include <string.h>
+
+#include <vector>
+
+namespace fhll {
+
+struct Launch {
+    const void* fn = nullptr;
+    uint32_t grid[3] = {1, 1, 1}, block[3] = {1, 1, 1};
+    uint32_t lds = 0;
+    uint32_t arg_off = 0, arg_bytes = 0;
+};
+
+struct LaunchList {
+    std::vector<Launch> v;
+    std::vector<unsigned char> args;
+    void clear() { v.clear(); args.clear(); }
+    bool empty() const { return v.empty(); }
+    size_t size() const { return v.size(); }
+    void add(const void* fn, uint32_t gx, uint32_t gy, uint32_t gz, uint32_t bx, uint32_t by, uint32_t bz, uint32_t lds, const void* kernarg, size_t bytes) {
+        Launch l;
+        l.fn = fn; l.grid[0] = gx; l.grid[1] = gy; l.grid[2] = gz; l.block[0] = bx; l.block[1] = by; l.block[2] = bz; l.lds = lds;
+        l.arg_off = (uint32_t)((args.size() + 15) & ~(size_t)15); l.arg_bytes = (uint32_t)bytes;
+        args.resize((size_t)l.arg_off + bytes, 0);
+        if (bytes) memcpy(args.data() + l.arg_off, kernarg, bytes);
+        v.push_back(l);
+    }
+    const unsigned char* arg(size_t i) const { return args.data() + v[i].arg_off; }
+    unsigned char* arg(size_t i) { return args.data() + v[i].arg_off; }
+};
+
+enum Diff : int { SAME = 0, PARAMS = 1, REBUILD = 2 };
+static inline Diff compare(const LaunchList& held, const LaunchList& now, std::vector<uint32_t>& changed) {
+    changed.clear();
+    if (held.size() != now.size()) return REBUILD;
+    for (size_t i = 0; i < now.size(); i++) {
+        const Launch &a = held.v[i], &b = now.v[i];
+        if (a.fn != b.fn || a.lds != b.lds || a.arg_bytes != b.arg_bytes || memcmp(a.block, b.block, sizeof(a.block))) { changed.clear(); return REBUILD; }
+        if (memcmp(a.grid, b.grid, sizeof(a.grid)) || (a.arg_bytes && memcmp(held.arg(i), now.arg(i), a.arg_bytes))) changed.push_back((uint32_t)i);
+    }
+    return changed.empty() ? SAME : PARAMS;
+}
+
+static const uint32_t MAX_CHANGED = 4, DROP_YOUNG = 8, MAX_STREAK = 64;
+enum Action : int {
+    DIRECT = 0,
+    DIRECT_DROP = 1,
+    BUILD = 2,
+    REPLAY = 3,
+    UPDATE = 4,
+};
+struct Policy {
+    uint32_t streak = 0;
+    uint32_t need = 2;
+    uint32_t replays = 0;
+    uint32_t young = 0;
+};
+static inline Action decide(Policy& p, bool have_graph, bool have_held, Diff d, size_t n_changed, size_t n_launches) {
+    if (!n_launches) return DIRECT;
+    if (!have_held || d == REBUILD) {
+        if (have_graph) {
+            if (p.replays < DROP_YOUNG) { if (++p.young >= 2) p.need = p.need * 2 > MAX_STREAK ? MAX_STREAK : p.need * 2; }
+            else { p.young = 0; p.need = 2; }
+        }
+        p.streak = 1; p.replays = 0;
+        return have_graph ? DIRECT_DROP : DIRECT;
+    }
+    p.streak++;
+    if (!have_graph) {
+        if (p.streak < p.need) return DIRECT;
+        p.replays = 0;
+        return BUILD;
+    }
+    if (d == PARAMS && n_changed > MAX_CHANGED) return DIRECT;
+    p.replays++;
+    if (p.replays == DROP_YOUNG) { p.young = 0; p.need = 2; }
+    return d == SAME ? REPLAY : UPDATE;
+}
+
+}
diff --git a/include/fidget_hip_debug.h b/include/fidget_hip_debug.h
--- a/include/fidget_hip_debug.h
+++ b/include/fidget_hip_debug.h
@@ -12,6 +12,7 @@
 uint32_t fhip_debug_leaves(fhip_ctx* ctx, void* out, uint32_t cap);
 fhip_status fhip_debug_probe(fhip_ctx* ctx, float* out);
 uint64_t fhip_debug_lane_frames(const fhip_ctx* ctx);
+void fhip_debug_lane_graph(const fhip_ctx* ctx, uint64_t out[4]);
 uint64_t fhip_debug_rare_frames(const fhip_ctx* ctx);
 int fhip_debug_lane_tune(const fhip_ctx* ctx, float ms[3], int* lanes);
 fhip_status fhip_debug_trans_probe(fhip_ctx* ctx, uint32_t copy, uint32_t fn, uint32_t first, uint64_t n, uint64_t out[2]);
```

After: 9.758 million Mvoxel/s. About the same (-0.0%).
